# HuiGuanLab/Lite-MKD

Hardware: AMD Instinct MI355X
Metric: episodes/sec (5-way 5-shot, 8x224^2 frames) (higher is better)
Workload: dtype f32

## Files before the change

include/lmkd.h:

```cpp
#ifndef LMKD_H
#define LMKD_H
#ifdef __cplusplus
extern "C" {
#endif

int lmkd_abi_version(void);
const char* lmkd_last_error(void);
int lmkd_device_check(int device);
int lmkd_set_activation_dtype(int mode);
int lmkd_get_activation_dtype(void);

int lmkd_gemm_f32(char layA, char layB, int M, int N, int K, float alpha, const float* A, long lda, long sA,
                  const float* B, long ldb, long sB, float beta, float* C, long ldc, long sC, const float* bias,
                  int relu, int batch, void* stream);
int lmkd_gemm_set_mode(int mode);
int lmkd_gemm_set_tile(int t);
long lmkd_gemm_ticket_words(void);
int lmkd_gemm_f32_splitk(char layA, char layB, int M, int N, int K, float alpha, const float* A, long lda, long sA,
                         const float* B, long ldb, long sB, float beta, float* C, long ldc, long sC, const float* bias,
                         int relu, int batch, void* workspace, long ws_bytes, unsigned* tickets, void* stream);

long lmkd_conv2d_packed_weight_elems(int Cout, int Cin, int Cs, int KH, int KW, int mode);
int lmkd_conv2d_pack_weights(const float* w_oihw, float* wp, int Cout, int Cin, int Cs, int KH, int KW, int mode ,
                             void* stream);
int lmkd_conv2d_fwd_row_tiles(int N, int H, int W, int Cout, int KH, int KW, int stride, int pad);
int lmkd_conv2d_fwd_row_tiles_cs(int N, int H, int W, int Cs, int Cout, int KH, int KW, int stride, int pad);
int lmkd_set_elementwise_wg_per_cu(int n);
int lmkd_conv_set_compute_dtype(int mode);
typedef struct lmkd_amax_desc {
  const void* x_words;
  const void* dy_words;
  void* out_words;
  const void* ref_words;
  int flags;
} lmkd_amax_desc;
#define LMKD_AMAX_FENCED 1
int lmkd_h2_fence_eval(const void* const* words, void* const* refs, int n, int* flags, void* stream);
long lmkd_conv_h2_fallbacks(void);
int lmkd_amax(const float* x, long n, void* word, void* stream);
long lmkd_amax_words(void);
long lmkd_conv2d_plane_elems(int ncols, int Kp);
long lmkd_conv_h2_launches(void);
int lmkd_conv2d_repack_multi(const float* const* ws, void* const* wfs, const int* dims, int n, void* stream);
int lmkd_conv2d_split_weights(const float* wp, void* wf, int ncols, int Kp, void* stream);
int lmkd_conv_get_compute_dtype(void);
int lmkd_conv_set_wgrad_planes(int on);
int lmkd_conv_set_patch(int on);
int lmkd_conv_set_stem_patch(int on);
int lmkd_conv_set_s2_patch(int on);
int lmkd_conv_set_wgrad_win16(int on);
int lmkd_conv_set_wgrad_stem(int on);
int lmkd_conv_set_wgrad_window(int on);
int lmkd_conv_set_patch16(int on);
int lmkd_conv_set_persistent(int on);
int lmkd_conv_set_xcd_mode(int mode);
int lmkd_conv_set_tile(int id);
int lmkd_conv2d_fwd(const float* x, const float* wp_fwd, float* y, float* stat_partial, int N, int H, int W, int Cs, int Cout,
                    int KH, int KW, int stride, int pad, void* stream);
int lmkd_conv2d_fwd_pre(const float* x_raw, const float* pre_stats, const float* wp_fwd, float* y, float* stat_partial, int N, int H,
                        int W, int Cs, int Cout, int KH, int KW, int stride, int pad, void* stream);
int lmkd_conv2d_fwd_bn(const float* x, const float* wp_fwd, float* y, const float* bn_stats, const float* res , int relu,
                       int N, int H, int W, int Cs, int Cout, int KH, int KW, int stride, int pad, void* stream,
                       const lmkd_amax_desc* amax );
int lmkd_conv2d_bwd_data(const float* dy, const float* wp_dgrad, float* dx, int N, int H, int W, int Cin, int Cout, int KH, int KW,
                         int stride, int pad, int accumulate, void* stream);
int lmkd_conv2d_bwd_data_bn_tiles(int N, int H, int W, int Cin, int Cout, int KH, int KW, int stride, int pad);
int lmkd_conv2d_bwd_data_bn(const float* dy, const float* wp_dgrad, float* dx, const float* bn_x, const float* bn_stats, float* part,
                            int N, int H, int W, int Cin, int Cout, int KH, int KW, int stride, int pad, void* stream);
long lmkd_conv2d_bwd_weight_workspace(int N, int H, int W, int Cs, int Cout, int KH, int KW, int stride, int pad);
int lmkd_conv2d_bwd_weight(const float* x, const float* dy, float* dw_oihw, float* workspace, long ws_bytes, int N, int H, int W,
                           int Cs, int Cin, int Cout, int KH, int KW, int stride, int pad, void* stream);
int lmkd_conv2d_bwd_weight_pre(const float* x_raw, const float* pre_stats, const float* dy, float* dw_oihw, float* workspace,
                               long ws_bytes, int N, int H, int W, int Cs, int Cin, int Cout, int KH, int KW, int stride, int pad,
                               void* stream);

int lmkd_conv2d_plan(int kind, int N, int H, int W, int Cs, int Cin, int Cout, int KH, int KW, int stride, int pad, int* info_host);

int lmkd_conv2d_bwd_weight_acc(const float* x, const float* pre_stats, const float* dy, float* dw_oihw, float* workspace, long ws_bytes,
                               int N, int H, int W, int Cs, int Cin, int Cout, int KH, int KW, int stride, int pad, void* stream);

int lmkd_frames_u8_to_nhwc4(const unsigned char* src, float* dst, const int* crop_y, const int* crop_x, const int* flip, int F, int Hs,
                            int Ws, int H, int W, int frames_per_video, void* stream);
int lmkd_resize_plan(int in_size, int out_size, int* bounds_host, int* coeffs_host);
int lmkd_resize_pass_u8(const unsigned char* src, unsigned char* dst, const int* bounds_dev, const int* coeffs_dev, int ksize, long outer,
                        int n_in, int n_out, long inner, void* stream);
int lmkd_frames_resize_crop_nhwc4(const unsigned char* src, float* dst, const int* bounds_h, const int* coeffs_h, int ksize_h,
                                  const int* bounds_v, const int* coeffs_v, int ksize_v, const int* crop_y, const int* crop_x,
                                  const int* flip, int F, int Hs, int Ws, int Hr, int Wr, int H, int W, int frames_per_video, void* stream);
long lmkd_jpeg_desc_bytes(void);
long lmkd_jpeg_pool_bytes(int n);
const char* lmkd_jpeg_reason(int reason);
int lmkd_jpeg_plan(const unsigned char* data, const long long* offsets, int n, void* descs, void* pool, long pool_cap, long long* info,
                   long long* totals);
int lmkd_jpeg_decode(const unsigned char* data, const void* descs, const void* pool, int n, short* coef, unsigned char* planes,
                     unsigned char* out, int* status, long long max_blocks, long long max_pixels, void* stream);
int lmkd_jpeg_decode_host(const unsigned char* data, const void* descs, const void* pool, int n, short* coef, unsigned char* planes,
                          unsigned char* out, int* status);
int lmkd_nchw3_to_nhwc4(const float* x_nchw, float* y_nhwc4, int N, int H, int W, void* stream, void* amax_words);
long lmkd_ticket_words(void);
int lmkd_bn_finalize(const float* partial, int T, int C, long count, const float* gamma, const float* beta, float* running_mean,
                     float* running_var, float momentum, float eps, float* stats, double* scratch, unsigned* tickets, void* stream,
                     const lmkd_amax_desc* amax );
int lmkd_bn_running_update(float* running_mean, float* running_var, const float* stats, int C, float momentum, void* stream);
int lmkd_bn_running_update_multi(float* const* running_mean, float* const* running_var, const float* const* stats_first,
                                 const float* const* stats_second, const int* C, int n, float momentum, void* stream);
int lmkd_bn_running_update_multi_nbt(float* const* running_mean, float* const* running_var, const float* const* stats_first,
                                     const float* const* stats_second, long long* const* num_batches_tracked, const int* C, int n,
                                     float momentum, void* stream);
int lmkd_bn_eval_stats(int C, const float* gamma, const float* beta, const float* running_mean, const float* running_var, float eps,
                       float* stats, void* stream);
int lmkd_bn_apply(const float* x, const float* stats, const float* res, const float* rstats, float* y, long rows, int C, int relu,
                  int res_mode, unsigned* mask_bits, void* stream);
long lmkd_bn_bwd_workspace(int C);
int lmkd_bn_backward(const float* dy, const float* x, const float* yact, const float* stats, const float* gamma, float* dx,
                     float* g_out, float* dgamma, float* dbeta, float* coef, void* workspace, unsigned* tickets, long rows, int C,
                     int mask_mode, int accumulate_param_grads, void* stream);
int lmkd_bn_backward_part(const float* part, int T, const float* dy, const float* x, const float* stats, const float* gamma, float* dx,
                          float* dgamma, float* dbeta, float* coef, void* workspace, unsigned* tickets, long rows, int C,
                          int accumulate_param_grads, void* stream);
int lmkd_relu_backward(const float* dy, const float* y, float* g, long n, void* stream);
int lmkd_bn_relu_maxpool_fwd(const float* x, const float* stats, float* y, unsigned char* idx, float* cmax, int N, int H, int W, int C,
                             void* stream);
int lmkd_maxpool_bwd(const float* dy, const unsigned char* idx, float* g, int N, int H, int W, int C, void* stream);
int lmkd_bn_backward_stats(const float* dy, const float* cmax, const float* stats, const float* gamma, float* dgamma, float* dbeta,
                           float* coef, void* workspace, unsigned* tickets, long pooled_rows, long count, int C, int accumulate_param_grads,
                           void* stream);
int lmkd_stem_unpool_bn_bwd(const float* dy, const unsigned char* idx, const float* c, const float* stats, const float* coef, float* dc,
                            int N, int H, int W, int C, void* stream, const lmkd_amax_desc* amax );
int lmkd_adaptive_maxpool_mean_fwd(const float* x, float* y, int F, int H, int W, int C, void* stream);
int lmkd_adaptive_maxpool_mean_bwd(const float* x, const float* dy, float* dx, int F, int H, int W, int C, void* stream);
long lmkd_colsum_workspace(int C);
int lmkd_colsum(const float* a, const float* b, float* out, long rows, int C, int accumulate, void* workspace, unsigned* tickets,
                void* stream);

long lmkd_mnv3_stat_tiles(long pixels);
int lmkd_dw_conv_fwd(const float* x, const float* w, float* y, float* stat_partial, int N, int H, int W, int C, int K, int stride, void* stream);
int lmkd_dw_conv_bwd_data(const float* dy, const float* w, float* dx, int N, int H, int W, int C, int K, int stride, void* stream);
long lmkd_dw_conv_bwd_weight_workspace(int N, int H, int W, int C, int K, int stride);
int lmkd_dw_conv_bwd_weight(const float* x, const float* dy, float* dw, void* workspace, long ws_bytes, int N, int H, int W, int C, int K,
                            int stride, int accumulate, void* stream);
int lmkd_col_stats(const float* x, float* stat_partial, long rows, int C, void* stream);
int lmkd_bn_act_fwd(const float* x, const float* stats, const float* res, float* y, long rows, int C, int act, void* stream);
long lmkd_bn_act_bwd_workspace(long rows, int C);
int lmkd_bn_act_bwd(const float* dy, const float* x, const float* stats, const float* gamma, float* dx, float* dparams, void* workspace,
                    long ws_bytes, long rows, int C, int act, void* stream);
int lmkd_se_mean(const float* a, float* m, int N, int HW, int C, void* stream);
int lmkd_se_scale_fwd(const float* a, const float* s, float* y, int N, int HW, int C, void* stream);
int lmkd_se_scale_bwd(const float* dy, const float* a, const float* s, const float* dm, float* da, float* ds, int N, int HW, int C, void* stream);
int lmkd_hardsigmoid_fwd(const float* x, float* y, long n, void* stream);
int lmkd_hardsigmoid_bwd(const float* dy, const float* x, float* dx, long n, void* stream);
int lmkd_stem3x3_fwd(const float* x4, const float* w, float* y, float* stat_partial, int N, int H, int W, void* stream);
long lmkd_stem3x3_bwd_weight_workspace(int N, int H, int W);
int lmkd_stem3x3_bwd_weight(const float* x4, const float* dy, float* dw, void* workspace, long ws_bytes, int N, int H, int W, int accumulate,
                            void* stream);

int lmkd_dropout_mask(float* mask, long n, float p, unsigned long long seed, void* stream);
int lmkd_dropout_mask_dev(float* mask, long n, float p, const unsigned long long* seed_dev, void* stream);
int lmkd_add_pe(const float* x, const float* pe, const float* mask, float* y, long rows, int D, int L, void* stream);
int lmkd_mul(const float* a, const float* b, float* out, long n, void* stream);
int lmkd_axpby(const float* x, float* y, float alpha, float beta, long n, void* stream);
int lmkd_trx_tuple_ln_fwd(const float* P, const float* bk, const float* bv, const float* gamma, const float* beta, const int* rowmap,
                          float* Kn, float* Khat, float* V, float* rstd, int NV, int L, int D, float eps, void* stream);
int lmkd_layernorm_bwd_rows(float* dK_inout, const float* Khat, const float* rstd, const float* gamma, long rows, int D, void* stream);
int lmkd_trx_tuple_bwd_gather(const float* dKraw, const float* dV, const int* rowmap, float* dP, int NV, int L, int D, void* stream);
int lmkd_segment_softmax_fwd(float* S, long rows, long ld, int nseg, const int* seg_off, const int* seg_cnt, void* stream);
int lmkd_segment_softmax_bwd(const float* P, float* dP_inout, long rows, long ld, int nseg, const int* seg_off, const int* seg_cnt,
                             void* stream);
int lmkd_trx_dist_fwd(const float* Qv, const float* proto, float* logits, int Nq, int way, int T, int D, int nseg, const int* seg_col,
                      void* stream);
int lmkd_trx_dist_bwd(const float* Qv, float* proto_inout, const float* g, float* dQv, int Nq, int way, int T, int D, int nseg,
                      const int* seg_col, void* stream);
int lmkd_trx_sup_sim_fwd(const float* proto, const int* seg_col, float* sim, float* gram, int Nq, int way, int nseg, int T, int D,
                         void* stream);
int lmkd_trx_sup_sim_bwd(const float* proto, const int* seg_col, const float* gram, const float* dsim, float* dproto, int Nq, int way,
                         int nseg, int T, int D, void* stream);
long lmkd_supportdk_workspace(int way);
int lmkd_supportdk_fwd(const float* support, float* out, int way, int shot, int seq_len, int D, void* workspace, void* stream);
int lmkd_supportdk_bwd(const float* support, const float* g, float* dsupport, int way, int shot, int seq_len, int D, void* stream);
int lmkd_mean_frames(const float* x, float* y, long nv, int L, int D, void* stream);
int lmkd_mean_frames_bwd(const float* dy, float* dx, long nv, int L, int D, void* stream);
int lmkd_edist_fwd(const float* qm, const float* sm, const int* sup_class, float* dist, float* logits, int Nq, int Ns, int way, int D,
                   void* stream);
int lmkd_edist_bwd(const float* qm, const float* sm, const int* sup_class, const float* dist, const float* g, float* dqm, float* dsm,
                   int Nq, int Ns, int way, int D, void* stream);

int lmkd_layernorm_fwd(const float* x, const float* res, long res_rows, const float* gamma, const float* beta, float* y, long ldy,
                       long rows, int D, float eps, void* stream);
int lmkd_mha_small(const float* qkv, float* out, int B, int L, int D, int H, void* stream);

int lmkd_d2m_loss(const float* s_kl, const float* t_kl, const float* s_ce, const long long* labels, const float* s_sup,
                  const float* t_sup, int Rq, int C, int Rs, int Cs, float T, float w_kl, float w_sup, float w_ce, float* out4,
                  float* g_kl, float* g_ce, float* g_sup, void* stream);
long lmkd_mse_loss_workspace(void);
int lmkd_mse_loss(const float* s, const float* t, long n, float* out1, float* grad, void* workspace, void* stream);
int lmkd_accuracy(const float* l1, const float* l2, const long long* labels, long long* pred, float* acc, int R, int C, void* stream);
int lmkd_sgd_step(float* param, float* grad, float lr, long n, int zero_grad, void* stream);
int lmkd_adam_step(float* param, float* grad, float* exp_avg, float* exp_avg_sq, float lr, float beta1, float beta2, float eps,
                   long step, long n, int zero_grad, void* stream);
int lmkd_fill(float* p, float v, long n, void* stream);

int lmkd_conv2d_fwd_row_tiles_seg(int N, int H, int W, int Cs, int Cout, int KH, int KW, int stride, int pad, int seg_n0, int* tiles0 );
int lmkd_conv2d_fwd_seg(const float* x, const float* pre_stats , const float* wp, float* y,
                        float* stat_partial, int N, int H, int W, int Cs, int Cout, int KH, int KW, int stride, int pad, int seg_n0, void* stream,
                        const lmkd_amax_desc* amax );
int lmkd_conv2d_bwd_data_bn_tiles_seg(int N, int H, int W, int Cin, int Cout, int KH, int KW, int stride, int pad, int seg_n0, int* tiles0 );
// ... 47 lines not shown
```

lite-mkd_amd/csrc/capi.hip:

```cpp
#include "common.h"
#include <stdarg.h>

static thread_local char g_err[512] = "";

extern "C" void lmkd_set_error(const char* fmt, ...) {
  va_list ap;
  va_start(ap, fmt);
  vsnprintf(g_err, sizeof(g_err), fmt, ap);
  va_end(ap);
}

extern "C" const char* lmkd_last_error(void) { return g_err; }

extern "C" int lmkd_abi_version(void) { return 3; }

extern "C" int lmkd_device_check(int device) {
  hipDeviceProp_t p;
  hipError_t e = hipGetDeviceProperties(&p, device);
  if (e != hipSuccess) {
    lmkd_set_error("lmkd_device_check: %s", hipGetErrorString(e));
    return LMKD_EHIP;
  }
  if (strncmp(p.gcnArchName, "gfx950", 6) != 0) {
    lmkd_set_error("lmkd_device_check: device %d is %s, this library is built for gfx950 only", device, p.gcnArchName);
    return LMKD_EINVAL;
  }
  return LMKD_OK;
}

int g_lmkd_act_bf16 = 0;
extern "C" int lmkd_set_activation_dtype(int mode) {
  LMKD_REQUIRE(mode == 0 || mode == 1, "lmkd_set_activation_dtype: 0 = fp32, 1 = bf16");
  g_lmkd_act_bf16 = mode;
  return LMKD_OK;
}
extern "C" int lmkd_get_activation_dtype(void) { return g_lmkd_act_bf16; }
```

lite-mkd_amd/csrc/conv.hip:

```cpp
#include "gemm_core.h"
#include <atomic>
#include <mutex>

struct ConvGemmArgs {
  const float* src;
  const float* wpk;
  float* out;
  float* stat_partial;
  int N, Hs, Ws, Cs;
  int Hr, Wr, rows_per_class, tiles_per_class;
  int sh;
  int Ho, Wo, Co, omul;
  int Kp, cps, nclass;
  int n_rt, n_ct, xcd_mode;
  int taps_pm1;
  int grid_step;
  int grid_total;
  int same;
  int halo;
  int accum;
  const float* ep_stats;
  const float* ep_res;
  int ep_relu;
  const float* pre_stats;
// ... 1226 lines not shown
  ConvGemmArgs a;
  fwd_geometry(a, N, H, W, Cs, Cout, KH, KW, stride, pad, seg_n0);
  const ConvPlan p = plan_fwd(a, KH, KW, pad);
  if (tiles0) *tiles0 = p.seg_t0;
  return p.tiles_per_class;
}
extern "C" int lmkd_conv2d_fwd_row_tiles(int N, int H, int W, int Cout, int KH, int KW, int stride, int pad) {
  return lmkd_conv2d_fwd_row_tiles_cs(N, H, W, 32, Cout, KH, KW, stride, pad);
}

static int conv2d_fwd_impl(const float* x, const float* wp, float* y, float* stat_partial, const float* ep_stats,
                           const float* ep_res, int ep_relu, int N, int H, int W, int Cs, int Cout, int KH, int KW, int stride,
                           int pad, void* stream, const float* pre_stats = nullptr, int seg_n0 = 0, const lmkd_amax_desc* am = nullptr) {
  LMKD_REQUIRE(x && wp && y, "lmkd_conv2d_fwd: null pointer");
  if (seg_n0 <= 0 || seg_n0 >= N) seg_n0 = 0;
  LMKD_REQUIRE(!seg_n0 || (conv_planes() && !ep_stats), "lmkd_conv2d_fwd_seg: two frame segments exist in the bf16-plane modes (training / plain forward)");
  LMKD_REQUIRE(aligned16(x) && aligned16(wp), "lmkd_conv2d_fwd: x / packed weights must be 16-byte aligned");
  LMKD_REQUIRE(Cs % 32 == 0 || Cs == 4, "lmkd_conv2d_fwd: channel count %d must be 4 (padded stem) or a multiple of 32", Cs);
  LMKD_REQUIRE(N > 0 && H > 0 && W > 0 && Cout > 0, "lmkd_conv2d_fwd: empty tensor");
  const bool smallc = Cs == 4;
  const int KWp = kw_padded(Cs, KW);
  LMKD_REQUIRE(!smallc || KWp == 8, "lmkd_conv2d_fwd: padded-stem path needs KW <= 8");
  LMKD_REQUIRE(KH * (smallc ? 1 : KW) <= LMKD_MAX_TAPS, "lmkd_conv2d_fwd: kernel %dx%d has too many taps", KH, KW);
  LMKD_REQUIRE(H < 32768 && W < 32768, "lmkd_conv2d_fwd: spatial dims too large");
  const bool act16 = g_lmkd_act_bf16;
  LMKD_REQUIRE(!pre_stats || (stat_partial && !smallc && !act16),
               "lmkd_conv2d_fwd_pre: the fused BatchNorm+ReLU loader exists for the training forward with fp32 activations (stat_partial given, Cs %% 32 == 0)");
  LMKD_REQUIRE(!act16 || (conv_nprod() == 1 && !ep_stats), "bf16 activations need lmkd_conv_set_compute_dtype(1) (training / plain forward)");
  const int Ho = conv_out(H, KH, stride, pad), Wo = conv_out(W, KW, stride, pad);
  LMKD_REQUIRE(Ho > 0 && Wo > 0, "lmkd_conv2d_fwd: empty output");
  LMKD_REQUIRE((long)N * H * W * Cs < 2147483647L && (long)N * Ho * Wo * Cout < 2147483647L,
               "lmkd_conv2d_fwd: tensor exceeds 2^31 elements");
  LMKD_REQUIRE(!conv_planes() || (long)N * H * W * Cs * (act16 && Cs != 4 ? 2 : 4) < 0xffffffe0L,
               "lmkd_conv2d_fwd: input tensor exceeds the 4 GiB buffer range of the bf16-plane kernels");
  ConvGemmArgs a;
  fwd_geometry(a, N, H, W, Cs, Cout, KH, KW, stride, pad, seg_n0);
  a.src = x; a.wpk = wp; a.out = y; a.stat_partial = stat_partial;
  a.h2_xw = am ? (const unsigned*)am->x_words : nullptr;
  a.amax_out = am ? (unsigned*)am->out_words : nullptr;
  note_fenced(am);
  a.ep_stats = ep_stats; a.ep_res = ep_res; a.ep_relu = ep_relu;
  a.pre_stats = pre_stats;
  const ConvPlan p = plan_fwd(a, KH, KW, pad);
  if (p.src2) {
    LMKD_REQUIRE((long)N * H * W * Cs * 4 < 2147483647L, "lmkd_conv2d_fwd: input tensor exceeds the 2 GiB offset range of the stride-2 patch form");
    fwd_src2_args(a, W, KWp);
  }
  int rc = launch_conv(a, p, (hipStream_t)stream);
  if (rc == LMKD_OK && a.amax_out && p.amax_pass) {
    const long per = (long)Ho * Wo * Cout, n0 = seg_n0 ? seg_n0 * per : (long)N * per;
    rc = amax_impl(y, n0, a.amax_out, 1, stream, false);
    if (rc == LMKD_OK && seg_n0) rc = amax_impl(y + n0, (long)N * per - n0, a.amax_out + LMKD_AMAX_SEG_WORDS, 1, stream, false);
  }
  return rc;
}

extern "C" int lmkd_conv2d_fwd(const float* x, const float* wp, float* y, float* stat_partial, int N, int H, int W, int Cs,
                               int Cout, int KH, int KW, int stride, int pad, void* stream) {
  return conv2d_fwd_impl(x, wp, y, stat_partial, nullptr, nullptr, 0, N, H, W, Cs, Cout, KH, KW, stride, pad, stream);
}

extern "C" int lmkd_conv2d_fwd_seg(const float* x, const float* pre_stats, const float* wp, float* y, float* stat_partial, int N, int H, int W,
                                   int Cs, int Cout, int KH, int KW, int stride, int pad, int seg_n0, void* stream, const lmkd_amax_desc* amax) {
  return conv2d_fwd_impl(x, wp, y, stat_partial, nullptr, nullptr, 0, N, H, W, Cs, Cout, KH, KW, stride, pad, stream, pre_stats, seg_n0, amax);
}

extern "C" int lmkd_conv2d_fwd_pre(const float* x_raw, const float* pre_stats, const float* wp, float* y, float* stat_partial, int N,
                                   int H, int W, int Cs, int Cout, int KH, int KW, int stride, int pad, void* stream) {
  LMKD_REQUIRE(pre_stats, "lmkd_conv2d_fwd_pre: BatchNorm table of the input missing");
  return conv2d_fwd_impl(x_raw, wp, y, stat_partial, nullptr, nullptr, 0, N, H, W, Cs, Cout, KH, KW, stride, pad, stream, pre_stats);
}

extern "C" int lmkd_conv2d_fwd_bn(const float* x, const float* wp, float* y, const float* bn_stats, const float* res, int relu,
                                  int N, int H, int W, int Cs, int Cout, int KH, int KW, int stride, int pad, void* stream, const lmkd_amax_desc* amax) {
  LMKD_REQUIRE(bn_stats, "lmkd_conv2d_fwd_bn: BatchNorm table missing");
  LMKD_REQUIRE(!g_lmkd_act_bf16, "lmkd_conv2d_fwd_bn: fp32 tensors only (with bf16 tensors run lmkd_conv2d_fwd + lmkd_bn_apply)");
  LMKD_REQUIRE(!conv_planes() || Cs % 32 == 0, "lmkd_conv2d_fwd_bn: the bf16-plane modes need Cs %% 32 == 0 (Cs=%d)", Cs);
  return conv2d_fwd_impl(x, wp, y, nullptr, bn_stats, res, relu, N, H, W, Cs, Cout, KH, KW, stride, pad, stream, nullptr, 0, amax);
}

static int bwd_data_args(ConvGemmArgs& a, const float* dy, const float* wd, float* dx, int N, int H, int W, int Cin, int Cout, int KH, int KW,
                         int stride, int pad, int accumulate, int seg_n0 = 0, const lmkd_amax_desc* am = nullptr) {
  if (seg_n0 <= 0 || seg_n0 >= N) seg_n0 = 0;
  LMKD_REQUIRE(!seg_n0 || conv_planes(), "lmkd_conv2d_bwd_data_seg: two frame segments exist in the bf16-plane modes");
  LMKD_REQUIRE(Cout % 32 == 0, "lmkd_conv2d_bwd_data: Cout=%d must be a multiple of 32", Cout);
  LMKD_REQUIRE(stride == 1 || stride == 2, "lmkd_conv2d_bwd_data: stride %d unsupported", stride);
  LMKD_REQUIRE(KH * KW <= LMKD_MAX_TAPS, "lmkd_conv2d_bwd_data: kernel too large");
  LMKD_REQUIRE(!g_lmkd_act_bf16 || conv_nprod() == 1, "bf16 activations need lmkd_conv_set_compute_dtype(1)");
  const int Ho = conv_out(H, KH, stride, pad), Wo = conv_out(W, KW, stride, pad);
  LMKD_REQUIRE((long)N * H * W * Cin < 2147483647L && (long)N * Ho * Wo * Cout < 2147483647L,
               "lmkd_conv2d_bwd_data: tensor exceeds 2^31 elements");
  LMKD_REQUIRE(!conv_planes() || (long)N * Ho * Wo * Cout * (g_lmkd_act_bf16 ? 2 : 4) < 0xffffffe0L,
               "lmkd_conv2d_bwd_data: dy exceeds the 4 GiB buffer range of the bf16-plane kernels");
  dgrad_geometry(a, N, H, W, Cin, Cout, KH, KW, stride, pad, seg_n0);
  a.src = dy; a.wpk = wd; a.out = dx; a.accum = accumulate;
  a.h2_xw = am ? (const unsigned*)am->dy_words : nullptr;
  return LMKD_OK;
}

extern "C" int lmkd_conv2d_bwd_data(const float* dy, const float* wd, float* dx, int N, int H, int W, int Cin, int Cout,
                                    int KH, int KW, int stride, int pad, int accumulate, void* stream) {
  LMKD_REQUIRE(dy && wd && dx, "lmkd_conv2d_bwd_data: null pointer");
  LMKD_REQUIRE(aligned16(dy) && aligned16(wd), "lmkd_conv2d_bwd_data: operands must be 16-byte aligned");
  ConvGemmArgs a;
  if (const int rc = bwd_data_args(a, dy, wd, dx, N, H, W, Cin, Cout, KH, KW, stride, pad, accumulate)) return rc;
  return launch_conv(a, plan_dgrad(a), (hipStream_t)stream);
}

extern "C" int lmkd_conv2d_bwd_data_bn_tiles_seg(int N, int H, int W, int Cin, int Cout, int KH, int KW, int stride, int pad, int seg_n0, int* tiles0) {
  if (stride != 1 || Cout % 32 != 0 || KH * KW > LMKD_MAX_TAPS) return 0;
  ConvGemmArgs a;
  if (bwd_data_args(a, nullptr, nullptr, nullptr, N, H, W, Cin, Cout, KH, KW, stride, pad, 0, seg_n0)) return 0;
  const ConvPlan p = plan_dgrad(a);
  if (!p.bnb_form) return 0;
  if (tiles0) *tiles0 = p.seg_t0;
  return p.tiles_per_class;
}
extern "C" int lmkd_conv2d_bwd_data_bn_tiles(int N, int H, int W, int Cin, int Cout, int KH, int KW, int stride, int pad) {
  return lmkd_conv2d_bwd_data_bn_tiles_seg(N, H, W, Cin, Cout, KH, KW, stride, pad, 0, nullptr);
}
extern "C" int lmkd_conv2d_bwd_data_seg(const float* dy, const float* wd, float* dx, const float* bn_x, const float* bn_stats, float* part, int N,
                                        int H, int W, int Cin, int Cout, int KH, int KW, int stride, int pad, int accumulate, int seg_n0, void* stream,
                                        const lmkd_amax_desc* amax) {
  LMKD_REQUIRE(dy && wd && dx, "lmkd_conv2d_bwd_data_seg: null pointer");
  LMKD_REQUIRE(aligned16(dy) && aligned16(wd), "lmkd_conv2d_bwd_data_seg: operands must be 16-byte aligned");
  LMKD_REQUIRE((bn_x != nullptr) == (bn_stats != nullptr) && (bn_x != nullptr) == (part != nullptr), "lmkd_conv2d_bwd_data_seg: bn_x, bn_stats and part go together");
  ConvGemmArgs a;
  if (const int rc = bwd_data_args(a, dy, wd, dx, N, H, W, Cin, Cout, KH, KW, stride, pad, accumulate, seg_n0, amax)) return rc;
  note_fenced(amax);
  if (bn_x) {
    LMKD_REQUIRE(!accumulate && aligned16(bn_x) && aligned16(bn_stats), "lmkd_conv2d_bwd_data_seg: the fused BatchNorm sums need a plain (non-accumulating) launch and aligned operands");
    a.bnb_x = bn_x; a.bnb_stats = bn_stats; a.stat_partial = part;
  }
  const ConvPlan p = plan_dgrad(a);
  LMKD_REQUIRE(!bn_x || p.bnb_form, "lmkd_conv2d_bwd_data_seg: this launch has no fused form (lmkd_conv2d_bwd_data_bn_tiles_seg returned 0)");
  return launch_conv(a, p, (hipStream_t)stream);
}
extern "C" int lmkd_conv2d_bwd_data_bn(const float* dy, const float* wd, float* dx, const float* bn_x, const float* bn_stats, float* part,
                                       int N, int H, int W, int Cin, int Cout, int KH, int KW, int stride, int pad, void* stream) {
  LMKD_REQUIRE(dy && wd && dx && bn_x && bn_stats && part, "lmkd_conv2d_bwd_data_bn: null pointer");
  LMKD_REQUIRE(aligned16(dy) && aligned16(wd) && aligned16(bn_x) && aligned16(bn_stats), "lmkd_conv2d_bwd_data_bn: operands must be 16-byte aligned");
  ConvGemmArgs a;
  if (const int rc = bwd_data_args(a, dy, wd, dx, N, H, W, Cin, Cout, KH, KW, stride, pad, 0)) return rc;
  a.bnb_x = bn_x; a.bnb_stats = bn_stats; a.stat_partial = part;
  const ConvPlan p = plan_dgrad(a);
  LMKD_REQUIRE(p.bnb_form, "lmkd_conv2d_bwd_data_bn: this launch has no fused form (lmkd_conv2d_bwd_data_bn_tiles returned 0)");
  return launch_conv(a, p, (hipStream_t)stream);
}

static int g_wgrad_planes = 1;
extern "C" int lmkd_conv_set_wgrad_planes(int on) { g_wgrad_planes = on ? 1 : 0; return LMKD_OK; }
static int g_wgrad_win16 = 1;
extern "C" int lmkd_conv_set_wgrad_win16(int on) { g_wgrad_win16 = on ? 1 : 0; return LMKD_OK; }
static int g_wgrad_window = 1;
extern "C" int lmkd_conv_set_wgrad_window(int on) { g_wgrad_window = on < 0 ? 0 : on; return LMKD_OK; }
static inline bool wgrad_win_eligible(int W, int Cs, int Cout, int KH, int KW, int stride, int pad) {
  return g_wgrad_window && g_wgrad_planes && conv_planes() && KH == 3 && KW == 3 && stride == 1 && pad == 1 &&
         Cs % 32 == 0 && 32 + 2 * (W + 1) <= 256;
}
static void wgrad_win_plan(int Mpix, int W, int Cs, int Cout, int* cob, int* splits, int* steps_per_split) {
  *cob = Cout >= 128 ? 4 : 2;
  const int tiles = cdiv(Cout, 32 * *cob) * (Cs / 32);
  const int steps = cdiv(Mpix, LMKD_BK);
  const int warm = cdiv(2 * (W + 1), LMKD_BK);
  const int resident = 256 * ((conv_nprod() >= 6 && *cob == 2) ? 2 : 8 / *cob);
  int sp = g_wgrad_window > 1 ? cdiv(g_wgrad_window, tiles)
                              : std::max((int)(((long)resident * steps + 19600L * 4 / *cob) / (39200L * 4 / *cob)), cdiv(128, tiles));
  const int cap = std::max(1, steps / (12 * warm));
  if (sp > cap) sp = cap;
  *steps_per_split = cdiv(steps, sp);
  *splits = cdiv(steps, *steps_per_split);
}

static void wgrad_plan(int Mpix, int Cout, int Kp, int* splits, int* steps_per_split, int* bm, int* bn, bool planes = false) {
  *bm = Cout <= 64 ? 64 : 128;
  *bn = (Kp % 128 == 0 && Kp >= 1024) ? 128 : 64;
  int per_cu = (*bm == 128 && *bn == 128) ? 2 : ((*bm == 64 && *bn == 64) ? 4 : 3);
  if (planes) {
    if (*bm == 64 && *bn == 128) *bn = 64;
    const int npl = conv_nprod() == 1 ? 1 : 3;
    const long lds = 1L * npl * LMKD_BK * ((*bm * 2 + 64) + (*bn * 2 + 64));
    per_cu = (int)(160 * 1024 / lds);
    if (per_cu > 4) per_cu = 4;
    if (per_cu < 1) per_cu = 1;
  }
  const int tiles = cdiv(Cout, *bm) * cdiv(Kp, *bn);
  const int steps = cdiv(Mpix, LMKD_BK);
  const int slots = 256 * per_cu;
  int best_sp = 1;
  double best_cost = 1e30;
  for (int r = 1; r <= 3; ++r) {
    int sp = (slots * r) / tiles;
    if (sp > steps / 4) sp = steps / 4;
    if (sp < 1) sp = 1;
    const int sps = cdiv(steps, sp);
    sp = cdiv(steps, sps);
    const double rounds = (double)cdiv((long)tiles * sp, slots);
    const double cost = rounds * sps + 1.0 * sp / 8.0;
    if (cost < best_cost) { best_cost = cost; best_sp = sp; }
  }
  if (planes && *bm == 64 && *bn == 64 && best_sp < cdiv(steps, 64)) best_sp = cdiv(steps, 64);
  *steps_per_split = cdiv(steps, best_sp);
  *splits = cdiv(steps, *steps_per_split);
}

static int g_wgrad_stem = 1;
extern "C" int lmkd_conv_set_wgrad_stem(int on) { g_wgrad_stem = on ? 1 : 0; return LMKD_OK; }
static int stem_wgrad_plan(int N, int H, int W, int Cs, int Cout, int KH, int KW, int stride, int pad, int* G) {
  if (!g_wgrad_stem || !g_wgrad_planes || conv_nprod(g_lmkd_act_bf16) < 6 || Cs != 4 || Cout != 64 || KH != 7 || KW != 7 || stride != 2 || pad != 3) return 0;
  const int Ho = conv_out(H, KH, stride, pad), Wo = conv_out(W, KW, stride, pad);
  if (Wo < 17 || Wo > 128 || W > 2 * Wo || Ho < 1) return 0;
  const int units = N * cdiv(Ho, 2);
  int g = std::max(1, 2048 / (2 * Wo));
  g = std::min(g, std::max(1, units / 256));
  *G = g;
  return cdiv(units, g);
}

enum class WgFam : unsigned char {
  Stem,
  Win16,
  Win,
  Planes,
  Tile,
};
struct WgradPlan {
  WgFam fam;
  bool pre, act16, smallc;
  int nprod;
  int bm, bn;
  int cob;
  int G;
  int splits, splits0, sps0, sps1, seg_pix0;
  int xcd;
  int grid;
  long need;
  long ws;
};

static long wgrad_workspace(int N, int H, int W, int Cs, int Cout, int KH, int KW, int stride, int pad) {
  const int Ho = conv_out(H, KH, stride, pad), Wo = conv_out(W, KW, stride, pad);
  const int Kp = KH * kw_padded(Cs, KW) * Cs;
  int G, splits, sps, bm, bn;
  if (const int slabs = stem_wgrad_plan(N, H, W, Cs, Cout, KH, KW, stride, pad, &G)) return (long)slabs * Cout * Kp * sizeof(float);
  wgrad_plan(N * Ho * Wo, Cout, Kp, &splits, &sps, &bm, &bn, conv_planes() && g_wgrad_planes);
  if (wgrad_win_eligible(W, Cs, Cout, KH, KW, stride, pad)) {
    int cob, wsplits, wsps;
    wgrad_win_plan(N * Ho * Wo, W, Cs, Cout, &cob, &wsplits, &wsps);
    splits = std::max(splits, wsplits);
  }
  return (long)splits * Cout * Kp * sizeof(float);
}

static WgradPlan plan_wgrad(int N, int H, int W, int Cs, int Cout, int KH, int KW, int stride, int pad, int seg_n0, bool pre, bool maxima) {
  WgradPlan p;
  memset(&p, 0, sizeof(p));
  const bool act16 = g_lmkd_act_bf16;
  const int Ho = conv_out(H, KH, stride, pad), Wo = conv_out(W, KW, stride, pad);
  const int Kp = KH * kw_padded(Cs, KW) * Cs, Mpix = N * Ho * Wo;
  p.pre = pre; p.act16 = act16; p.smallc = Cs == 4;
  p.ws = wgrad_workspace(N, H, W, Cs, Cout, KH, KW, stride, pad);
  if (seg_n0)
    p.ws = std::max(p.ws, wgrad_workspace(seg_n0, H, W, Cs, Cout, KH, KW, stride, pad) + wgrad_workspace(N - seg_n0, H, W, Cs, Cout, KH, KW, stride, pad));
  p.seg_pix0 = seg_n0 ? seg_n0 * Ho * Wo : Mpix;
  if (const int slabs = stem_wgrad_plan(N, H, W, Cs, Cout, KH, KW, stride, pad, &p.G)) {
    p.fam = WgFam::Stem;
    p.nprod = conv_nprod(false, maxima);
    p.splits = p.grid = slabs;
  } else if (wgrad_win_eligible(W, Cs, Cout, KH, KW, stride, pad)) {
    const bool w16 = g_wgrad_win16 && conv_nprod(act16) >= 6;
    p.fam = w16 ? WgFam::Win16 : WgFam::Win;
    p.nprod = w16 ? conv_nprod(false, maxima) : conv_nprod(act16);
    wgrad_win_plan(Mpix, W, Cs, Cout, &p.cob, &p.splits, &p.sps0);
    p.splits0 = p.splits;
    if (seg_n0) {
      int sp1, cob1;
      wgrad_win_plan(p.seg_pix0, W, Cs, Cout, &p.cob, &p.splits0, &p.sps0);
      wgrad_win_plan(Mpix - p.seg_pix0, W, Cs, Cout, &cob1, &sp1, &p.sps1);
      p.splits = p.splits0 + sp1;
    }
    p.grid = 8 * cdiv(p.splits, 8) * cdiv(Cout, 32 * p.cob) * (Cs / 32);
  } else {
    const bool planes = conv_planes() && g_wgrad_planes;
    p.fam = planes ? WgFam::Planes : WgFam::Tile;
    p.nprod = planes ? conv_nprod(act16, maxima && !p.smallc && !pre) : (conv_nprod() == 1 ? 1 : 0);
    wgrad_plan(Mpix, Cout, Kp, &p.splits, &p.sps0, &p.bm, &p.bn, planes);
    p.splits0 = p.splits;
    if (seg_n0) {
      int sp1, bm1, bn1;
      wgrad_plan(p.seg_pix0, Cout, Kp, &p.splits0, &p.sps0, &p.bm, &p.bn, planes);
      wgrad_plan(Mpix - p.seg_pix0, Cout, Kp, &sp1, &p.sps1, &bm1, &bn1, planes);
      p.splits = p.splits0 + sp1;
    }
    p.xcd = (g_xcd_mode != 0 && g_xcd_mode != 1 && p.splits >= 32) ? 1 : 0;
    p.grid = (p.xcd ? 8 * cdiv(p.splits, 8) : p.splits) * cdiv(Cout, p.bm) * cdiv(Kp, p.bn);
  }
  p.need = (long)p.splits * Cout * Kp * sizeof(float);
  return p;
}

template <int NPROD, int D, int RLC>
static void launch_stem_wgrad(const StemWgradArgs& w, dim3 grid, size_t lds, hipStream_t s) {
  lds_attr_once<stem_wgrad_kernel<NPROD, D, RLC>>(160 * 1024);
  hipLaunchKernelGGL((stem_wgrad_kernel<NPROD, D, RLC>), grid, dim3(512), lds, s, w);
}
template <int NPROD>
static void launch_stem_wgrad(const StemWgradArgs& w, dim3 grid, size_t lds, hipStream_t s) {
  const bool deep = cdiv(2 * w.Wo, 32) >= 6;
  if (deep && w.RL == 1856) launch_stem_wgrad<NPROD, 6, 1856>(w, grid, lds, s);
  else if (deep) launch_stem_wgrad<NPROD, 6, 0>(w, grid, lds, s);
  else launch_stem_wgrad<NPROD, 2, 0>(w, grid, lds, s);
}
template <int COB>
static void launch_wgrad_win(const WgradWinArgs& w, const WgradPlan& p, bool big, hipStream_t s) {
  const dim3 grid(p.grid);
  if (p.fam == WgFam::Win16) {
    constexpr int JW = COB == 2 ? 1 : 2;
    constexpr int NT = 64 * COB * (2 / JW);
    with_nprod<3, 6, 9>(p.nprod, [&](auto np) {
      if (big && p.pre) hipLaunchKernelGGL((conv_wgrad_win16_kernel<COB, np, 256, true, 9, JW>), grid, dim3(NT), 0, s, w);
      else if (big) hipLaunchKernelGGL((conv_wgrad_win16_kernel<COB, np, 256, false, 9, JW>), grid, dim3(NT), 0, s, w);
      else if (p.pre) hipLaunchKernelGGL((conv_wgrad_win16_kernel<COB, np, 128, true, 9, JW>), grid, dim3(NT), 0, s, w);
      else hipLaunchKernelGGL((conv_wgrad_win16_kernel<COB, np, 128, false, 9, JW>), grid, dim3(NT), 0, s, w);
    });
    return;
  }
  auto go = [&](auto np, auto a16, auto pre) {
    constexpr int NPROD = decltype(np)::value;
    constexpr bool A16 = decltype(a16)::value, PRE = decltype(pre)::value;
    constexpr int TPW = (COB == 2 && NPROD != 1) ? 5 : 9;
    constexpr int NT = 64 * COB * ((9 + TPW - 1) / TPW);
    if (big) hipLaunchKernelGGL((conv_wgrad_win_kernel<COB, NPROD, A16, 256, PRE, TPW>), grid, dim3(NT), 0, s, w);
    else hipLaunchKernelGGL((conv_wgrad_win_kernel<COB, NPROD, A16, 128, PRE, TPW>), grid, dim3(NT), 0, s, w);
  };
  using T = std::true_type;
  using F = std::false_type;
  if (p.act16) go(std::integral_constant<int, 1>{}, T{}, F{});
  else with_nprod<1, 6, 9>(p.nprod, [&](auto np) { if (p.pre) go(np, F{}, T{}); else go(np, F{}, F{}); });
}

template <class CFG>
static void launch_wgrad_planes(const WgradArgs& a, const WgradPlan& p, hipStream_t s) {
  const dim3 grid(p.grid), block(256);
  if (p.act16) {
    if (p.smallc) hipLaunchKernelGGL((conv_wgrad_x3_kernel<CFG, true, 1, false, true>), grid, block, 0, s, a);
    else hipLaunchKernelGGL((conv_wgrad_x3_kernel<CFG, false, 1, false, true>), grid, block, 0, s, a);
  } else if (p.smallc) {
    with_nprod<1, 6, 9>(p.nprod, [&](auto np) { hipLaunchKernelGGL((conv_wgrad_x3_kernel<CFG, true, np, false>), grid, block, 0, s, a); });
  } else if (p.pre) {
    with_nprod<1, 6, 9>(p.nprod, [&](auto np) { hipLaunchKernelGGL((conv_wgrad_x3_kernel<CFG, false, np, true>), grid, block, 0, s, a); });
  } else {
    with_nprod<1, 3, 6, 9>(p.nprod, [&](auto np) { hipLaunchKernelGGL((conv_wgrad_x3_kernel<CFG, false, np, false>), grid, block, 0, s, a); });
  }
}

template <class CFG, bool SM, int THR>
static void launch_wgrad_tile(const WgradArgs& a, const WgradPlan& p, hipStream_t s) {
  const dim3 grid(p.grid);
  if (p.nprod == 1) hipLaunchKernelGGL((conv_wgrad_kernel<CFG, SM, true>), grid, dim3(THR), 0, s, a);
  else if (!SM && p.pre) hipLaunchKernelGGL((conv_wgrad_kernel<CFG, false, false, true>), grid, dim3(THR), 0, s, a);
  else hipLaunchKernelGGL((conv_wgrad_kernel<CFG, SM, false>), grid, dim3(THR), 0, s, a);
}

static int conv2d_bwd_weight_impl(const float* x, const float* pre_stats, const float* dy, float* dw_oihw, float* workspace,
                                  long ws_bytes, int N, int H, int W, int Cs, int Cin, int Cout, int KH, int KW, int stride, int pad,
                                  void* stream, int accumulate = 0, int seg_n0 = 0, const lmkd_amax_desc* am = nullptr) {
  const unsigned* amax_x = am ? (const unsigned*)am->x_words : nullptr;
  const unsigned* amax_dy = am ? (const unsigned*)am->dy_words : nullptr;
  note_fenced(am);
  LMKD_REQUIRE(x && dy && dw_oihw && workspace, "lmkd_conv2d_bwd_weight: null pointer");
  if (seg_n0 <= 0 || seg_n0 >= N) seg_n0 = 0;
  LMKD_REQUIRE(aligned16(x) && aligned16(dy) && aligned16(workspace), "lmkd_conv2d_bwd_weight: operands must be 16-byte aligned");
  LMKD_REQUIRE(Cs % 32 == 0 || Cs == 4, "lmkd_conv2d_bwd_weight: channel count %d must be 4 or a multiple of 32", Cs);
  LMKD_REQUIRE(Cout % 4 == 0, "lmkd_conv2d_bwd_weight: Cout %% 4 != 0");
  const bool smallc = Cs == 4;
  const WgradPlan p = plan_wgrad(N, H, W, Cs, Cout, KH, KW, stride, pad, seg_n0, pre_stats != nullptr, amax_x && amax_dy);
  LMKD_REQUIRE(!seg_n0 || p.fam != WgFam::Tile, "lmkd_conv2d_bwd_weight_seg: two frame segments exist in the bf16-plane modes");
  LMKD_REQUIRE(!pre_stats || (!smallc && (conv_nprod() != 1 || p.fam != WgFam::Tile) && !p.act16), "lmkd_conv2d_bwd_weight_pre: Cs %% 32 == 0, fp32 activations only");
  LMKD_REQUIRE(!p.act16 || (conv_nprod() == 1 && p.fam != WgFam::Tile), "bf16 activations need lmkd_conv_set_compute_dtype(1) and the plane weight-gradient kernel");
  const int Ho = conv_out(H, KH, stride, pad), Wo = conv_out(W, KW, stride, pad);
  const int KWp = kw_padded(Cs, KW), Kp = KH * KWp * Cs, Mpix = N * Ho * Wo;
  LMKD_REQUIRE((long)N * H * W * Cs < 2147483647L && (long)Mpix * Cout < 2147483647L, "lmkd_conv2d_bwd_weight: tensor too large");
  LMKD_REQUIRE(ws_bytes >= p.need, "lmkd_conv2d_bwd_weight: workspace too small");
  hipStream_t s = (hipStream_t)stream;
  if (p.fam == WgFam::Stem) {
    LMKD_REQUIRE((long)Mpix * 64 * 4 < 0xffffffe0L && (long)N * H * W * 16 < 0xffffffe0L, "lmkd_conv2d_bwd_weight: tensor too large for 32-bit byte offsets");
    StemWgradArgs w;
    memset(&w, 0, sizeof(w));
    w.dy = dy; w.x = x; w.slab = workspace;
    w.h2_xw = amax_x; w.h2_dyw = amax_dy;
    w.N = N; w.H = H; w.W = W; w.Ho = Ho; w.Wo = Wo;
    w.upi = cdiv(Ho, 2); w.units = N * w.upi; w.G = p.G; w.slabs = p.splits;
    w.RL = 16 * Wo + 64;
    const size_t lds = (size_t)2 * 10 * 3 * w.RL + 2 * 3 * STEM_WG_APLANE;
    with_nprod<3, 6, 9>(p.nprod, [&](auto np) { launch_stem_wgrad<np>(w, dim3(p.grid), lds, s); });
    LMKD_CHECK_LAUNCH("stem_wgrad_kernel");
    if (Kp <= 256) {
      hipLaunchKernelGGL(wgrad_reduce_stem_kernel, dim3(Cout), dim3(256, 4), 0, s, (const float*)workspace, dw_oihw, p.splits, Cout, Cin, Cs, KH, KW,
                         KWp, Kp, accumulate);
    } else {
      launch_wgrad_reduce((const float*)workspace, dw_oihw, p.splits, Cout, Cin, Cs, KH, KW, KWp, Kp, accumulate, s);
    }
    LMKD_CHECK_LAUNCH("wgrad_reduce_kernel");
    return LMKD_OK;
  }
  if (p.fam == WgFam::Win16 || p.fam == WgFam::Win) {
    LMKD_REQUIRE((long)Mpix * std::max(Cs, Cout) * 4 < 2147483647L, "lmkd_conv2d_bwd_weight: tensor too large for 32-bit byte offsets");
    WgradWinArgs w;
    memset(&w, 0, sizeof(w));
    w.dy = dy; w.x = x; w.slab = workspace; w.pre_stats = pre_stats;
    w.h2_xw = amax_x; w.h2_dyw = amax_dy;
    w.N = N; w.H = H; w.W = W; w.Cs = Cs; w.Co = Cout; w.Kp = Kp; w.Mpix = Mpix;
    w.steps_total = cdiv(Mpix, LMKD_BK);
    w.splits = p.splits; w.steps_per_split = p.sps0;
    w.seg_pix0 = p.seg_pix0; w.seg_splits0 = p.splits0; w.sps1 = p.sps1;
    w.n_ct = cdiv(Cout, 32 * p.cob); w.n_it = Cs / 32;
    w.div_hw = make_fastdiv(H * W); w.div_w = make_fastdiv(W);
    const bool big = 32 + 2 * (W + 1) > 128;
    if (p.cob == 4) launch_wgrad_win<4>(w, p, big, s);
    else launch_wgrad_win<2>(w, p, big, s);
    LMKD_CHECK_LAUNCH("conv_wgrad_win_kernel");
    launch_wgrad_reduce((const float*)workspace, dw_oihw, p.splits, Cout, Cin, Cs, KH, KW, KWp, Kp, accumulate, s);
    LMKD_CHECK_LAUNCH("wgrad_reduce_kernel");
    return LMKD_OK;
  }
  WgradArgs a;
  memset(&a, 0, sizeof(a));
  a.dy = dy; a.x = x; a.slab = workspace; a.pre_stats = pre_stats;
  a.h2_xw = amax_x; a.h2_dyw = amax_dy;
  a.N = N; a.Hs = H; a.Ws = W; a.Cs = Cs;
  a.Ho = Ho; a.Wo = Wo; a.Co = Cout;
  a.stride = stride; a.pad = pad; a.KH = KH; a.KW = KW; a.KWp = KWp;
  a.Kp = Kp; a.Mpix = Mpix;
  a.steps_per_split = p.sps0;
  a.seg_pix0 = p.seg_pix0; a.seg_splits0 = p.splits0; a.sps1 = p.sps1;
  a.steps_total = cdiv(Mpix, LMKD_BK);
  a.div_hw = make_fastdiv(Ho * Wo); a.div_w = make_fastdiv(Wo);
  a.n_mt = cdiv(Cout, p.bm); a.n_jt = cdiv(Kp, p.bn); a.splits = p.splits;
  a.xcd_mode = p.xcd;
  const int bm = p.bm, bn = p.bn;
  LMKD_REQUIRE(!smallc || (bm == 64 && bn == 64), "lmkd_conv2d_bwd_weight: padded-stem path expects Cout <= 64");
  if (p.fam == WgFam::Planes) {
    if (bm == 128 && bn == 128) launch_wgrad_planes<WgCfg<128, 128, 2, 2>>(a, p, s);
    else if (bm == 128) launch_wgrad_planes<WgCfg<128, 64, 2, 2>>(a, p, s);
    else launch_wgrad_planes<WgCfg<64, 64, 2, 2>>(a, p, s);
    LMKD_CHECK_LAUNCH("conv_wgrad_x3_kernel");
  } else {
    if (smallc) launch_wgrad_tile<TileCfg<64, 64, 2, 2>, true, LMKD_THREADS>(a, p, s);
    else if (bm == 64 && bn == 64) launch_wgrad_tile<TileCfg<64, 64, 2, 2>, false, LMKD_THREADS>(a, p, s);
    else if (bm == 128 && bn == 64) launch_wgrad_tile<TileCfg<128, 64, 2, 2>, false, LMKD_THREADS>(a, p, s);
    else if (bm == 64 && bn == 128) launch_wgrad_tile<TileCfg<64, 128, 2, 2>, false, LMKD_THREADS>(a, p, s);
    else launch_wgrad_tile<TileCfg<128, 128, 2, 4>, false, 512>(a, p, s);
    LMKD_CHECK_LAUNCH("conv_wgrad_kernel");
  }
  launch_wgrad_reduce((const float*)workspace, dw_oihw, p.splits, Cout, Cin, Cs, KH, KW, KWp, Kp, accumulate, s);
  LMKD_CHECK_LAUNCH("wgrad_reduce_kernel");
  return LMKD_OK;
}

extern "C" long lmkd_conv2d_bwd_weight_workspace_seg(int N, int H, int W, int Cs, int Cout, int KH, int KW, int stride, int pad, int seg_n0) {
  if (seg_n0 <= 0 || seg_n0 >= N) seg_n0 = 0;
  return plan_wgrad(N, H, W, Cs, Cout, KH, KW, stride, pad, seg_n0, false, false).ws;
}
extern "C" long lmkd_conv2d_bwd_weight_workspace(int N, int H, int W, int Cs, int Cout, int KH, int KW, int stride, int pad) {
  return lmkd_conv2d_bwd_weight_workspace_seg(N, H, W, Cs, Cout, KH, KW, stride, pad, 0);
}

extern "C" int lmkd_conv2d_bwd_weight(const float* x, const float* dy, float* dw_oihw, float* workspace, long ws_bytes,
                                      int N, int H, int W, int Cs, int Cin, int Cout, int KH, int KW, int stride, int pad,
                                      void* stream) {
  return conv2d_bwd_weight_impl(x, nullptr, dy, dw_oihw, workspace, ws_bytes, N, H, W, Cs, Cin, Cout, KH, KW, stride, pad, stream);
}

extern "C" int lmkd_conv2d_bwd_weight_pre(const float* x_raw, const float* pre_stats, const float* dy, float* dw_oihw,
                                          float* workspace, long ws_bytes, int N, int H, int W, int Cs, int Cin, int Cout, int KH,
                                          int KW, int stride, int pad, void* stream) {
  LMKD_REQUIRE(pre_stats, "lmkd_conv2d_bwd_weight_pre: BatchNorm table of the input missing");
  return conv2d_bwd_weight_impl(x_raw, pre_stats, dy, dw_oihw, workspace, ws_bytes, N, H, W, Cs, Cin, Cout, KH, KW, stride, pad, stream);
}

extern "C" int lmkd_conv2d_bwd_weight_acc(const float* x, const float* pre_stats, const float* dy, float* dw_oihw, float* workspace,
                                          long ws_bytes, int N, int H, int W, int Cs, int Cin, int Cout, int KH, int KW, int stride,
                                          int pad, void* stream) {
  return conv2d_bwd_weight_impl(x, pre_stats, dy, dw_oihw, workspace, ws_bytes, N, H, W, Cs, Cin, Cout, KH, KW, stride, pad, stream, 1);
}


extern "C" int lmkd_conv2d_bwd_weight_seg(const float* x, const float* pre_stats, const float* dy, float* dw_oihw, float* workspace, long ws_bytes,
                                          int N, int H, int W, int Cs, int Cin, int Cout, int KH, int KW, int stride, int pad, int accumulate,
                                          int seg_n0, void* stream, const lmkd_amax_desc* amax) {
  return conv2d_bwd_weight_impl(x, pre_stats, dy, dw_oihw, workspace, ws_bytes, N, H, W, Cs, Cin, Cout, KH, KW, stride, pad, stream, accumulate, seg_n0, amax);
}

extern "C" int lmkd_conv2d_plan(int kind, int N, int H, int W, int Cs, int Cin, int Cout, int KH, int KW, int stride, int pad,
                                int* info) {
  LMKD_REQUIRE(info && kind >= 0 && kind <= 2, "lmkd_conv2d_plan: kind must be 0 (forward), 1 (data gradient) or 2 (weight gradient)");
  LMKD_REQUIRE(N > 0 && H > 0 && W > 0 && Cout > 0 && KH > 0 && KW > 0 && stride > 0, "lmkd_conv2d_plan: bad shape");
  if (kind == 2) {
    const WgradPlan p = plan_wgrad(N, H, W, Cs, Cout, KH, KW, stride, pad, 0, false, false);
    info[1] = p.xcd; info[2] = p.splits; info[3] = p.grid;
    switch (p.fam) {
      case WgFam::Stem: info[0] = 14; info[4] = 2; break;
      case WgFam::Win16:
      case WgFam::Win: info[0] = p.cob == 4 ? 5 : 6; info[1] = 1; info[4] = 1; break;
      default: info[0] = (p.bm == 128 && p.bn == 128) ? 1 : (p.bm == 128 ? 2 : (p.bn == 128 ? 4 : 3)); info[4] = 0; break;
    }
    return LMKD_OK;
  }
  ConvGemmArgs a;
  if (kind == 0) fwd_geometry(a, N, H, W, Cs, Cout, KH, KW, stride, pad, 0);
  else dgrad_geometry(a, N, H, W, Cin, Cout, KH, KW, stride, pad, 0);
  const ConvPlan p = kind == 0 ? plan_fwd(a, KH, KW, pad) : plan_dgrad(a);
  info[0] = p.tile; info[1] = p.xcd; info[2] = p.nclass; info[3] = p.grid;
  info[4] = p.fam == ConvFam::Stem ? 2 : (p.fam == ConvFam::Patch || p.fam == ConvFam::Patch16 || p.fam == ConvFam::Patch1p ? 1 : 0);
  return LMKD_OK;
}
```

lite-mkd_amd/csrc/conv_patch.h:

```cpp
#pragma once

#define PATCH_HALO_MAX 57

template <int NPL> struct PatchRow { static constexpr int BYTES = NPL == 1 ? 80 : (NPL == 2 ? 144 : 208); };

static inline size_t patch_lds_bytes(int bm, int halo, int npl) { return (size_t)(bm + 2 * halo + 1) * (npl == 1 ? 80 : (npl == 2 ? 144 : 208)); }

#ifdef LMKD_STAMPS
__device__ unsigned long long g_lmkd_stamps[4096 * 8];
#define STAMP(k) do { if (threadIdx.x == 0 && (blockIdx.x & 63) == 0 && (blockIdx.x >> 6) < 4096) g_lmkd_stamps[(blockIdx.x >> 6) * 8 + (k)] = __builtin_amdgcn_s_memtime(); } while (0)
#else
#define STAMP(k) do { } while (0)
#endif


template <class Cfg>
__device__ __forceinline__ void patch_h2_epilogue(const ConvGemmArgs& a, f32x16 (&acc)[Cfg::TM][Cfg::TN], const int* s_out, float* s_red, int rt,
                                                  int n0, int wm, int wn, int lane, int tid, int seg, int row0, int M, float h2_ix, float h2_iw) {
  const int cl0 = wn * (Cfg::TN * 32) + (lane & 31);
  const bool bnb = a.bnb_x != nullptr;
  float s1[Cfg::TN], s2[Cfg::TN];
  float amo = 0.f;
  const bool plain = a.nclass == 1;
  const int rows = M - row0 < Cfg::BM ? M - row0 : Cfg::BM;
// ... 170 lines not shown
  if (Lc < 0) return;
  u32x4 rp[NI];
  float4 psc = float4(), psh = float4();
  auto issue_patch = [&](const PatchTile& d, int cc) {
#pragma unroll
    for (int i = 0; i < NI; ++i)
      if (i * RPP < P) rp[i] = __builtin_amdgcn_raw_buffer_load_b128(prs, ((d.p_ok >> i) & 1u) ? d.p_off0 + i * p_step + (unsigned)(cc * 32 * ESZ) : X3_OOB, 0, 0);
    if (PRE) {
      const float* pre_tab = a.pre_stats + (long)d.seg * 5 * a.Cs;
      psc = *reinterpret_cast<const float4*>(pre_tab + 2 * a.Cs + cc * 32 + pk);
      psh = *reinterpret_cast<const float4*>(pre_tab + 3 * a.Cs + cc * 32 + pk);
    }
  };
  for (int j = tid; j < ROWB / 4; j += Cfg::THREADS) reinterpret_cast<unsigned*>(psm + (long)P * ROWB)[j] = 0u;
  int it = 0;
  bool requested = false;
  for (;;) {
    PSTAMP(0);
    const int Ln = PERSIST ? next_tile(Lc + a.grid_step, nxt) : -1;
    const int ntap = cur.ntap;
    const Tap* taps = s_args.taps[cur.cls];
    const int ph = cur.cls >> 1, pw = cur.cls & 1;
    const int M = cur.mend, row0 = cur.row0, n0 = cur.ct * Cfg::BN;
    const int nk = ntap * a.cps;
    const Tap my_tap = taps[lane < ntap ? lane : 0];
    if (!requested && nk > 0) issue_patch(cur, 0);
    requested = false;
    unsigned h2_xbits = 0u, h2_wbits = 0u;
    if constexpr (NPROD == 3) {
      h2_xbits = a.h2_xw[cur.seg * LMKD_AMAX_SEG_WORDS + (tid & (LMKD_AMAX_SLOTS - 1)) * LMKD_AMAX_STRIDE];
      h2_wbits = *reinterpret_cast<const unsigned*>(reinterpret_cast<const unsigned short*>(a.wpk) + (long)a.Co * a.Kp * 16);
    }
    LB lb;
    const bool neg = NPL == 3 && NPROD != 3 && x3_neg_tile(cur.ltile, cur.ltiles);
    if constexpr (NPROD == 3)
      lb.init(reinterpret_cast<const unsigned short*>(a.wpk) + (long)a.Co * a.Kp * 16 + 32, a.Co, a.Kp, n0 + wn * (Cfg::TN * 32), lane, false);
    else
      lb.init(a.wpk, a.Co, a.Kp, n0 + wn * (Cfg::TN * 32), lane, neg);
    u32x4 rb0[LB::NR], rb1[LB::NR];
    int b_tp = 0, b_cc = 0;
    if (nk > 0) {
      lb.load(__builtin_amdgcn_readlane(my_tap.kofs, 0), rb0);
      if (++b_tp == ntap) { b_tp = 0; ++b_cc; }
      if (nk > 1) {
        lb.load((ntap > 1 ? __builtin_amdgcn_readlane(my_tap.kofs, 1) : __builtin_amdgcn_readlane(my_tap.kofs, 0)) + b_cc * LMKD_BK, rb1);
        if (++b_tp == ntap) { b_tp = 0; ++b_cc; }
      }
    }
    const bool inv = PERSIST && a.nclass == 1;
    const bool tables = !inv || it == 0;
    if (tables && tid < ntap) {
      s_tap_shift[tid] = (my_tap.dh * a.Ws + my_tap.dw) * ROWB;
      s_tap_kofs[tid] = my_tap.kofs;
      s_tap_dhw[tid] = (my_tap.dh << 16) | (my_tap.dw & 0xffff);
    }
    if (tables && NPROD == 3 && a.taps_pm1 && tid < 64) {
      const int rb = tid & 7, cb = tid >> 3;
      unsigned m = 0;
      for (int tp = 0; tp < ntap; ++tp) {
        const int dh = taps[tp].dh, dw = taps[tp].dw;
        if (((rb >> (dh + 1)) & 1) && ((cb >> (dw + 1)) & 1)) m |= 1u << tp;
      }
      s_mask_lut[tid] = (unsigned short)m;
    }
    if (a.nclass != 1 || !(NPROD == 3)) {
      for (int r = tid; r < Cfg::BM; r += Cfg::THREADS) {
        const int m = row0 + r;
        int ob = -1;
        if (m < M) {
          if (a.nclass == 1) {
            ob = m * a.Co;
          } else {
            const int n = fdiv(m, a.div_hw);
            const int rem = m - n * a.Hs * a.Ws;
            const int aa = fdiv(rem, a.div_w), bb = rem - aa * a.Ws;
            const int oh = aa * a.omul + ph, ow = bb * a.omul + pw;
            if (oh < a.Ho && ow < a.Wo) ob = ((n * a.Ho + oh) * a.Wo + ow) * a.Co;
          }
        }
        s_out[r] = ob;
      }
    }
    if (tables) __syncthreads();
    unsigned a_base[Cfg::TM], a_mask[Cfg::TM];
    {
      int hh[Cfg::TM], ww[Cfg::TM];
#pragma unroll
      for (int i = 0; i < Cfg::TM; ++i) {
        const int r = a_row + 32 * i, m = row0 + r;
        a_base[i] = (unsigned)((r + halo) * ROWB + 16 * h);
        a_mask[i] = 0;
        hh[i] = -0x4000; ww[i] = 0;
        if (m < M) {
          const int n = fdiv(m, a.div_hw);
          const int rem = m - n * a.Hs * a.Ws;
          hh[i] = fdiv(rem, a.div_w);
          ww[i] = rem - hh[i] * a.Ws;
        }
      }
      if (NPROD == 3 && a.taps_pm1) {
#pragma unroll
        for (int i = 0; i < Cfg::TM; ++i) {
          const unsigned Hs = (unsigned)a.Hs, Ws = (unsigned)a.Ws;
          const unsigned rbits = ((unsigned)(hh[i] - 1) < Hs ? 1u : 0u) | ((unsigned)hh[i] < Hs ? 2u : 0u) | ((unsigned)(hh[i] + 1) < Hs ? 4u : 0u);
          const unsigned cbits = ((unsigned)(ww[i] - 1) < Ws ? 1u : 0u) | ((unsigned)ww[i] < Ws ? 2u : 0u) | ((unsigned)(ww[i] + 1) < Ws ? 4u : 0u);
          a_mask[i] = s_mask_lut[rbits | (cbits << 3)];
        }
      } else
      for (int t0 = 0; t0 < ntap; t0 += 9) {
        int dv[9];
#pragma unroll
        for (int q = 0; q < 9; ++q) dv[q] = s_tap_dhw[t0 + q < ntap ? t0 + q : 0];
#pragma unroll
        for (int q = 0; q < 9; ++q) {
          const int dh = dv[q] >> 16, dw = (int)(short)(dv[q] & 0xffff);
#pragma unroll
          for (int i = 0; i < Cfg::TM; ++i) {
            const int y = hh[i] + dh, x = ww[i] + dw;
            if (t0 + q < ntap && (unsigned)y < (unsigned)a.Hs && (unsigned)x < (unsigned)a.Ws) a_mask[i] |= 1u << (t0 + q);
          }
        }
      }
    }
    float h2_sx = 1.f, h2_ix = 1.f, h2_iw = 1.f;
    if constexpr (NPROD == 3) {
      unsigned v = h2_xbits;
#pragma unroll
      for (int o = 32; o >= 1; o >>= 1) {
        const unsigned u = (unsigned)__shfl_xor((int)v, o, 64);
        v = u > v ? u : v;
      }
      h2_sx = h2_scale(__builtin_amdgcn_readfirstlane(v));
      h2_ix = 1.f / h2_sx;
      h2_iw = 1.f / h2_scale(h2_wbits);
    }
    auto store_patch = [&]() {
#pragma unroll
      for (int i = 0; i < NI; ++i) {
        const int j = tid / LPR + RPP * i;
        if (j >= P) continue;
        unsigned char* d = psm + j * ROWB + pk * 2;
        if constexpr (IN16) {
          *reinterpret_cast<u32x4*>(d) = rp[i];
        } else {
          float4 v = make_float4(__uint_as_float(rp[i].x), __uint_as_float(rp[i].y), __uint_as_float(rp[i].z), __uint_as_float(rp[i].w));
          if (PRE && ((cur.p_ok >> i) & 1u)) {
            v.x = fmaxf(fmaf(v.x, psc.x, psh.x), 0.f); v.y = fmaxf(fmaf(v.y, psc.y, psh.y), 0.f);
            v.z = fmaxf(fmaf(v.z, psc.z, psh.z), 0.f); v.w = fmaxf(fmaf(v.w, psc.w, psh.w), 0.f);
          }
          if (NPL == 1) {
            *reinterpret_cast<uint2*>(d) = x3_round4(v);
          } else if constexpr (NPROD == 3) {
            uint2 q0, q1;
            h2_split4(v, h2_sx, q0, q1);
            *reinterpret_cast<uint2*>(d) = q0;
            *reinterpret_cast<uint2*>(d + 64) = q1;
          } else {
            uint2 q0, q1, q2;
            x3_split4(v, q0, q1, q2);
            *reinterpret_cast<uint2*>(d) = q0;
            *reinterpret_cast<uint2*>(d + 64) = q1;
            *reinterpret_cast<uint2*>(d + 128) = q2;
          }
        }
      }
    };
    f32x16 acc[Cfg::TM][Cfg::TN];
#pragma unroll
    for (int i = 0; i < Cfg::TM; ++i)
#pragma unroll
      for (int j = 0; j < Cfg::TN; ++j)
#pragma unroll
        for (int e = 0; e < 16; ++e) acc[i][j][e] = 0.f;
    auto issue_b = [&](u32x4 (&rb)[LB::NR]) {
      lb.load(s_tap_kofs[b_tp] + b_cc * LMKD_BK, rb);
      if (++b_tp == ntap) { b_tp = 0; ++b_cc; }
    };
    int k_tp = 0, k_cc = 0;
    constexpr bool PIPE = NPL == 1;
    bf16x8 avp0[2][NPL][Cfg::TM], avp1[2][NPL][Cfg::TM];
    auto read_tap = [&](int tp, bf16x8 (&dst)[2][NPL][Cfg::TM]) {
      const unsigned sh = (unsigned)s_tap_shift[tp];
#pragma unroll
      for (int i = 0; i < Cfg::TM; ++i) {
        const unsigned ad = ((a_mask[i] >> tp) & 1u) ? a_base[i] + sh : zero_addr;
#pragma unroll
        for (int g = 0; g < 2; ++g)
#pragma unroll
          for (int p = 0; p < NPL; ++p) dst[g][p][i] = *reinterpret_cast<const bf16x8*>(psm + ad + p * 64 + g * 32);
      }
    };
    auto step = [&](int t, u32x4 (&rb)[LB::NR], u32x4 (&rbn)[LB::NR], bf16x8 (&avc)[2][NPL][Cfg::TM], bf16x8 (&avn)[2][NPL][Cfg::TM]) {
      if (k_tp == 0) {
        if (!(inv && k_cc == 0)) __syncthreads();
        store_patch();
        __syncthreads();
        {
          const bool more = k_cc + 1 < a.cps;
          const bool ahead = PERSIST && !more && Ln >= 0 && nxt.ntap > 0;
          if (more || ahead) {
            PatchTile d;
            d.p_off0 = more ? cur.p_off0 : nxt.p_off0;
            d.p_ok = more ? cur.p_ok : nxt.p_ok;
            d.seg = more ? cur.seg : nxt.seg;
            issue_patch(d, more ? k_cc + 1 : 0);
            requested = ahead;
          }
        }
        if constexpr (PIPE) read_tap(0, avc);
      }
      if constexpr (PIPE) {
        if (k_tp + 1 < ntap) read_tap(k_tp + 1, avn);
        __builtin_amdgcn_sched_barrier(0);
#pragma unroll
        for (int g = 0; g < 2; ++g)
#pragma unroll
          for (int j = 0; j < Cfg::TN; ++j) {
            const bf16x8 b0 = x3_as_bf16(rb[j * 2 + g]);
#pragma unroll
            for (int i = 0; i < Cfg::TM; ++i) acc[i][j] = __builtin_amdgcn_mfma_f32_32x32x16_bf16(avc[g][0][i], b0, acc[i][j], 0, 0, 0);
          }
        if (++k_tp == ntap) { k_tp = 0; ++k_cc; }
        __builtin_amdgcn_sched_barrier(0);
        x3_landed(rbn);
        x3_landed(rp);
        __builtin_amdgcn_sched_barrier(0);
        if (t + 2 < nk) issue_b(rb);
        return;
      }
      const unsigned sh = (unsigned)s_tap_shift[k_tp];
      unsigned ad[Cfg::TM];
#pragma unroll
      for (int i = 0; i < Cfg::TM; ++i) ad[i] = ((a_mask[i] >> k_tp) & 1u) ? a_base[i] + sh : zero_addr;
      constexpr bool AHEAD = NPL * Cfg::TM < 12 && (Cfg::THREADS == 512 || NPL == 1);
      bf16x8 av[2][NPL][Cfg::TM];
      auto read_a = [&](int g) {
#pragma unroll
        for (int p = 0; p < NPU; ++p)
#pragma unroll
          for (int i = 0; i < Cfg::TM; ++i) av[AHEAD ? g : 0][p][i] = *reinterpret_cast<const bf16x8*>(psm + ad[i] + p * 64 + g * 32);
      };
      read_a(0);
      if (AHEAD) read_a(1);
      __builtin_amdgcn_sched_barrier(0);
#pragma unroll
      for (int g = 0; g < 2; ++g) {
        const int ga = AHEAD ? g : 0;
        if (!AHEAD && g == 1) {
          __builtin_amdgcn_sched_barrier(0);
          read_a(1);
          __builtin_amdgcn_sched_barrier(0);
        }
#pragma unroll
        for (int j = 0; j < Cfg::TN; ++j) {
          if constexpr (NPROD == 1) {
            const bf16x8 b0 = x3_as_bf16(rb[j * 2 + g]);
#pragma unroll
            for (int i = 0; i < Cfg::TM; ++i) acc[i][j] = __builtin_amdgcn_mfma_f32_32x32x16_bf16(av[ga][0][i], b0, acc[i][j], 0, 0, 0);
          } else if constexpr (NPROD == 3) {
            const f16x8 b0 = __builtin_bit_cast(f16x8, rb[j * 4 + g * 2 + 0]), b1 = __builtin_bit_cast(f16x8, rb[j * 4 + g * 2 + 1]);
#pragma unroll
            for (int i = 0; i < Cfg::TM; ++i) {
              f32x16 c = acc[i][j];
              c = __builtin_amdgcn_mfma_f32_32x32x16_f16(__builtin_bit_cast(f16x8, av[ga][0][i]), b1, c, 0, 0, 0);
              c = __builtin_amdgcn_mfma_f32_32x32x16_f16(__builtin_bit_cast(f16x8, av[ga][1][i]), b0, c, 0, 0, 0);
              c = __builtin_amdgcn_mfma_f32_32x32x16_f16(__builtin_bit_cast(f16x8, av[ga][0][i]), b0, c, 0, 0, 0);
              acc[i][j] = c;
            }
          } else {
            const bf16x8 b0 = x3_as_bf16(rb[j * 6 + g * 3 + 0]), b1 = x3_as_bf16(rb[j * 6 + g * 3 + 1]), b2 = x3_as_bf16(rb[j * 6 + g * 3 + 2]);
#pragma unroll
            for (int i = 0; i < Cfg::TM; ++i) {
              f32x16 c = acc[i][j];
              if (NPROD == 9) {
                c = __builtin_amdgcn_mfma_f32_32x32x16_bf16(av[ga][2][i], b2, c, 0, 0, 0);
                c = __builtin_amdgcn_mfma_f32_32x32x16_bf16(av[ga][1][i], b2, c, 0, 0, 0);
                c = __builtin_amdgcn_mfma_f32_32x32x16_bf16(av[ga][2][i], b1, c, 0, 0, 0);
              }
              c = __builtin_amdgcn_mfma_f32_32x32x16_bf16(av[ga][1][i], b1, c, 0, 0, 0);
              c = __builtin_amdgcn_mfma_f32_32x32x16_bf16(av[ga][0][i], b2, c, 0, 0, 0);
              c = __builtin_amdgcn_mfma_f32_32x32x16_bf16(av[ga][2][i], b0, c, 0, 0, 0);
              c = __builtin_amdgcn_mfma_f32_32x32x16_bf16(av[ga][0][i], b1, c, 0, 0, 0);
              c = __builtin_amdgcn_mfma_f32_32x32x16_bf16(av[ga][1][i], b0, c, 0, 0, 0);
              c = __builtin_amdgcn_mfma_f32_32x32x16_bf16(av[ga][0][i], b0, c, 0, 0, 0);
              acc[i][j] = c;
            }
          }
        }
      }
      if (++k_tp == ntap) { k_tp = 0; ++k_cc; }
      __builtin_amdgcn_sched_barrier(0);
      x3_landed(rbn);
      x3_landed(rp);
      __builtin_amdgcn_sched_barrier(0);
      if (t + 2 < nk) issue_b(rb);
    };
    PSTAMP(1);
    if (nk > 0) {
      x3_landed(rp);
      x3_landed(rb0);
      x3_landed(rb1);
      __builtin_amdgcn_sched_barrier(0);
      PSTAMP(2);
      int t = 0;
      for (; t + 1 < nk; t += 2) {
        step(t, rb0, rb1, avp0, avp1);
        step(t + 1, rb1, rb0, avp1, avp0);
// ... 18 lines not shown
```

lite-mkd_amd/csrc/conv_patch16.h:

```cpp
#pragma once
#ifndef LMKD_ABL
#define LMKD_ABL 0
#endif

__device__ __host__ __forceinline__ constexpr int patch16_kslot(int q) { return ((q & 1) << 1) | (q >> 1); }
__device__ __forceinline__ int patch16_pixel(int j) { return (j >= 4 && j < 12) ? 2 * (j - 4) : (j < 4 ? 2 * j + 1 : 2 * (j - 8) + 1); }

template <int CTRL>
__device__ __forceinline__ float dpp_add(float v) {
  return v + __int_as_float(__builtin_amdgcn_update_dpp(0, __float_as_int(v), CTRL, 0xf, 0xf, false));
}
__device__ __forceinline__ float row16_sum(float v) {
  v = dpp_add<0xB1>(v);
  v = dpp_add<0x4E>(v);
  v = dpp_add<0x141>(v);
  return dpp_add<0x140>(v);
}

template <int TN, int NPW = 3>
struct X3FragB16 {
  static constexpr int NT = 2 * TN;
  static constexpr int NR = NT * NPW;
  __amdgpu_buffer_rsrc_t rs;
  unsigned off[NT];
// ... 114 lines not shown
  constexpr int NPL = 3;
  constexpr int NPU = NPROD == 3 ? 2 : 3;
  constexpr int ROWB = PatchRow<NPL>::BYTES;
  constexpr int LPR = 8;
  constexpr int RPP = Cfg::THREADS / LPR;
  constexpr int NI = (Cfg::BM + 2 * PATCH_HALO_MAX + RPP - 1) / RPP;
  constexpr int NB = 2 * Cfg::TM, NC = 2 * Cfg::TN;
  using LB = X3FragB16<Cfg::TN, NPU>;
  extern __shared__ __attribute__((aligned(16))) unsigned char psm[];
  __shared__ int s_out[Cfg::BM];
  __shared__ int s_tap_kofs[LMKD_MAX_TAPS];
  static_assert(NB == 4 && PatchRow<NPL>::BYTES % 16 == 0 && PatchRow<NPL>::BYTES / 16 * (Cfg::BM + 2 * PATCH_HALO_MAX + 1) < 65536,
                "four 16-bit patch offsets (in units of 16 bytes) per lane and tap");
  __shared__ __attribute__((aligned(8))) unsigned short s_adp[LMKD_MAX_TAPS * Cfg::BM];
  __shared__ float s_red[Cfg::WM * Cfg::BN * 2];
  __shared__ int s_src[SRC2 ? Cfg::BM + 2 * PATCH_HALO_MAX : 1];
  const int tid = threadIdx.x;
  STAMP(0);
  int rt, ct;
  if (!xcd_decode(blockIdx.x, a.n_rt, a.n_ct, a.xcd_mode, rt, ct)) return;
  const int tile = rt / a.nclass;
  const int cls = rt - tile * a.nclass;
  const int ph = cls >> 1, pw = cls & 1;
  const int ntap = a.ntap[cls];
  if (a.accum && ntap == 0) return;
  const Tap* taps = a.taps[cls];
  const int halo = a.halo, P = Cfg::BM + 2 * halo;
  const SegTile sg = seg_tile(a, tile, Cfg::BM);
  const int M = sg.mend;
  const int row0 = sg.row0, n0 = ct * Cfg::BN;
  if (tid < ntap) {
    const Tap tp = taps[tid];
    s_tap_kofs[tid] = tp.kofs;
  }
  for (int r = tid; r < Cfg::BM; r += Cfg::THREADS) {
    const int m = row0 + r;
    int ob = -1;
    if (m < M) {
      if (a.nclass == 1) {
        ob = m * a.Co;
      } else {
        const int n = fdiv(m, a.div_hw);
        const int rem = m - n * a.Hs * a.Ws;
        const int aa = fdiv(rem, a.div_w), bb = rem - aa * a.Ws;
        const int oh = aa * a.omul + ph, ow = bb * a.omul + pw;
        if (oh < a.Ho && ow < a.Wo) ob = ((n * a.Ho + oh) * a.Wo + ow) * a.Co;
      }
    }
    s_out[r] = ob;
  }
  for (int j = tid; j < ROWB / 4; j += Cfg::THREADS) reinterpret_cast<unsigned*>(psm + (long)P * ROWB)[j] = 0u;
  if constexpr (SRC2) {
    for (int j = tid; j < P; j += Cfg::THREADS) {
      const int m = row0 - halo + j;
      int off = -1;
      if (m >= 0 && m < a.rows_per_class) {
        const int n = fdiv(m, a.div_hw);
        const int rem = m - n * a.Hs * a.Ws;
        const int aa = fdiv(rem, a.div_w), bb = rem - aa * a.Ws;
        off = (((n * 2 * a.Hs + 2 * aa) * a.s2_wfull + 2 * bb) * a.Cs) * 4;
      }
      s_src[j] = off;
    }
  }
  const int lane = tid & 63, wave = tid >> 6;
  float h2_sx = 1.f, h2_ix = 1.f, h2_iw = 1.f;
  bool h2_one = true;
  if constexpr (NPROD == 3) {
    h2_sx = h2_scale(amax_read(a.h2_xw, sg.seg));
    const float sw = h2_scale(*reinterpret_cast<const unsigned*>(reinterpret_cast<const unsigned short*>(a.wpk) + (long)a.Co * a.Kp * 16));
    h2_ix = 1.f / h2_sx;
    h2_iw = 1.f / sw;
    const int ex = (int)((__float_as_uint(h2_ix) >> 23) & 0xffu) + (int)((__float_as_uint(h2_iw) >> 23) & 0xffu) - 254;
    h2_one = ex >= -126 && ex <= 126;
    if (h2_one) h2_ix *= h2_iw;
  }
  const int wm = wave / Cfg::WN, wn = wave % Cfg::WN;
  const int kq = lane >> 4;
  const int ksl = patch16_kslot(kq);
  const int pxl = patch16_pixel(lane & 15);
  constexpr bool EARLY = !SRC2 && Cfg::BN == 64;
  if constexpr (!EARLY) {
    for (int r = tid; r < Cfg::BM; r += Cfg::THREADS) {
      const int m = row0 + r;
      const int within = r % (Cfg::TM * 32), px = within & 15;
      const int l16 = (px & 1) ? ((px >> 1) + (px < 8 ? 0 : 8)) : (px >> 1) + 4;
      unsigned short* dst = s_adp + ((r / (Cfg::TM * 32)) * 16 + l16) * NB + (within >> 4);
      int hh = -0x40000000, ww = 0;
      if (m < M) {
        const int n = fdiv(m, a.div_hw);
        const int rem = m - n * a.Hs * a.Ws;
        hh = fdiv(rem, a.div_w);
        ww = rem - hh * a.Ws;
      }
      for (int tp = 0; tp < ntap; ++tp) {
        const int y = hh + taps[tp].dh, x = ww + taps[tp].dw;
        const bool in = (unsigned)y < (unsigned)a.Hs && (unsigned)x < (unsigned)a.Ws;
        dst[tp * Cfg::BM] = (unsigned short)((in ? (r + halo + taps[tp].dh * a.Ws + taps[tp].dw) : P) * (ROWB / 16));
      }
    }
  }
  const unsigned lane_off = (unsigned)(16 * ksl);
  const unsigned short* adp_lane = s_adp + (wm * 16 + (lane & 15)) * NB;
  const __amdgpu_buffer_rsrc_t prs = x3_rsrc(a.src, (long)a.N * a.Hs * a.Ws * a.Cs * 4 * (SRC2 ? 4 : 1));
  const int pk = (tid & (LPR - 1)) * 4;
  const long pix0 = (long)row0 - halo + tid / LPR;
  const unsigned p_off0 = (unsigned)((pix0 * a.Cs + pk) * 4), p_step = (unsigned)(RPP * a.Cs * 4);
  unsigned p_ok = 0;
#pragma unroll
  for (int i = 0; i < NI; ++i) {
    const long pix = pix0 + RPP * i;
    if (tid / LPR + RPP * i < P && pix >= 0 && pix < (long)a.N * a.Hs * a.Ws) p_ok |= 1u << i;
  }
  u32x4 rp[NI];
  int k_cc_abl = 0;
  float4 psc = float4(), psh = float4();
  const float* pre_tab = PRE ? a.pre_stats + (long)sg.seg * 5 * a.Cs : nullptr;
  auto issue_patch = [&](int cc, int sc = 0) {
    if ((LMKD_ABL & 32) && cc > 0) return;
    if constexpr (SRC2) {
      const unsigned rel = (unsigned)((a.s2_off[sc] + cc * 32 + pk) * 4);
#pragma unroll
      for (int i = 0; i < NI; ++i) {
        if (i * RPP >= P) continue;
        const int j = tid / LPR + RPP * i;
        const int so = j < P ? s_src[j] : -1;
        rp[i] = __builtin_amdgcn_raw_buffer_load_b128(prs, so >= 0 ? (unsigned)so + rel : X3_OOB, 0, 0);
      }
      return;
    }
#pragma unroll
    for (int i = 0; i < NI; ++i)
      if (i * RPP < P) rp[i] = __builtin_amdgcn_raw_buffer_load_b128(prs, ((p_ok >> i) & 1u) ? p_off0 + i * p_step + (unsigned)(cc * 32 * 4) : X3_OOB, 0, 0);
    if (PRE) {
      psc = *reinterpret_cast<const float4*>(pre_tab + 2 * a.Cs + cc * 32 + pk);
      psh = *reinterpret_cast<const float4*>(pre_tab + 3 * a.Cs + cc * 32 + pk);
    }
  };
  auto store_patch = [&]() {
    if ((LMKD_ABL & 64) && k_cc_abl > 0) return;
#pragma unroll
    for (int i = 0; i < NI; ++i) {
      const int j = tid / LPR + RPP * i;
      if (j >= P) continue;
      unsigned char* d = psm + j * ROWB + pk * 2;
      float4 v = make_float4(__uint_as_float(rp[i].x), __uint_as_float(rp[i].y), __uint_as_float(rp[i].z), __uint_as_float(rp[i].w));
      if (PRE && ((p_ok >> i) & 1u)) {
        v.x = fmaxf(fmaf(v.x, psc.x, psh.x), 0.f); v.y = fmaxf(fmaf(v.y, psc.y, psh.y), 0.f);
        v.z = fmaxf(fmaf(v.z, psc.z, psh.z), 0.f); v.w = fmaxf(fmaf(v.w, psc.w, psh.w), 0.f);
      }
      uint2 q0, q1, q2;
      if constexpr (NPROD == 3) {
        if (LMKD_ABL & 4) { q0 = make_uint2(__float_as_uint(v.x), __float_as_uint(v.y)); q1 = make_uint2(__float_as_uint(v.z), __float_as_uint(v.w)); }
        else h2_split4(v, h2_sx, q0, q1);
      } else x3_split4(v, q0, q1, q2);
      *reinterpret_cast<uint2*>(d) = q0;
      *reinterpret_cast<uint2*>(d + 64) = q1;
      if (NPU == 3) *reinterpret_cast<uint2*>(d + 128) = q2;
    }
  };
  const bool neg = x3_neg_tile(sg.ltile, sg.ltiles);
  if (NPROD == 3 && neg) h2_ix = -h2_ix;
  LB lb;
  lb.init(a.wpk, a.Co, a.Kp, n0 + wn * (Cfg::TN * 32), lane, neg);
  f32x4 acc[NB][NC];
#pragma unroll
  for (int b = 0; b < NB; ++b)
#pragma unroll
    for (int c = 0; c < NC; ++c) acc[b][c] = f32x4{0.f, 0.f, 0.f, 0.f};
  const int nk = ntap * a.cps;
  u32x4 rb0[LB::NR], rb1[LB::NR];
  int b_tp = 0, b_cc = 0;
  auto issue_b = [&](u32x4 (&rb)[LB::NR]) {
    lb.load(s_tap_kofs[b_tp] + b_cc * LMKD_BK, rb);
    if (++b_tp == ntap) { b_tp = 0; ++b_cc; }
  };
  int k_tp = 0, k_cc = 0;
  int k_sc = 0;
  bf16x8 av[NPL][NB / 2];
  auto step = [&](int t, u32x4 (&rb)[LB::NR], u32x4 (&rbn)[LB::NR]) {
    if (SRC2 ? k_tp == a.s2_t0[k_sc] : k_tp == 0) {
      __syncthreads();
      store_patch();
      __syncthreads();
      if constexpr (SRC2) {
        if (k_sc + 1 < a.s2_ncls) issue_patch(k_cc, k_sc + 1);
        else if (k_cc + 1 < a.cps) issue_patch(k_cc + 1, 0);
      } else {
        if (k_cc + 1 < a.cps) issue_patch(k_cc + 1);
      }
    }
    const uint2 pk2 = *reinterpret_cast<const uint2*>(adp_lane + k_tp * Cfg::BM);
    const unsigned ad[NB] = {((pk2.x & 0xffffu) << 4) + lane_off, ((pk2.x >> 16) << 4) + lane_off, ((pk2.y & 0xffffu) << 4) + lane_off,
                             ((pk2.y >> 16) << 4) + lane_off};
    constexpr int HB = NB / 2;
    auto read_a = [&](int hf) {
      if ((LMKD_ABL & 2) && t > 0) return;
#pragma unroll
      for (int p = 0; p < NPU; ++p)
#pragma unroll
        for (int b = 0; b < HB; ++b) av[p][b] = *reinterpret_cast<const bf16x8*>(psm + ad[hf * HB + b] + p * 64);
    };
    read_a(0);
    __builtin_amdgcn_sched_barrier(0);
#pragma unroll
    for (int hf = 0; hf < 2; ++hf) {
      if (hf == 1) {
        __builtin_amdgcn_sched_barrier(0);
        read_a(1);
        __builtin_amdgcn_sched_barrier(0);
      }
#pragma unroll
      for (int c = 0; c < NC; ++c) {
        const bf16x8 w0 = x3_as_bf16(rb[c * NPU + 0]), w1 = x3_as_bf16(rb[c * NPU + 1]), w2 = x3_as_bf16(rb[c * NPU + (NPU - 1)]);
#pragma unroll
        for (int b = 0; b < HB; ++b) {
          f32x4 d = acc[hf * HB + b][c];
          if constexpr (NPROD == 3) {
            d = __builtin_amdgcn_mfma_f32_16x16x32_f16(__builtin_bit_cast(f16x8, w1), __builtin_bit_cast(f16x8, av[0][b]), d, 0, 0, 0);
            d = __builtin_amdgcn_mfma_f32_16x16x32_f16(__builtin_bit_cast(f16x8, w0), __builtin_bit_cast(f16x8, av[1][b]), d, 0, 0, 0);
            d = __builtin_amdgcn_mfma_f32_16x16x32_f16(__builtin_bit_cast(f16x8, w0), __builtin_bit_cast(f16x8, av[0][b]), d, 0, 0, 0);
            acc[hf * HB + b][c] = d;
            continue;
          }
          if (NPROD == 9) {
            d = __builtin_amdgcn_mfma_f32_16x16x32_bf16(w2, av[2][b], d, 0, 0, 0);
            d = __builtin_amdgcn_mfma_f32_16x16x32_bf16(w2, av[1][b], d, 0, 0, 0);
            d = __builtin_amdgcn_mfma_f32_16x16x32_bf16(w1, av[2][b], d, 0, 0, 0);
          }
          d = __builtin_amdgcn_mfma_f32_16x16x32_bf16(w1, av[1][b], d, 0, 0, 0);
          d = __builtin_amdgcn_mfma_f32_16x16x32_bf16(w2, av[0][b], d, 0, 0, 0);
          d = __builtin_amdgcn_mfma_f32_16x16x32_bf16(w0, av[2][b], d, 0, 0, 0);
          d = __builtin_amdgcn_mfma_f32_16x16x32_bf16(w1, av[0][b], d, 0, 0, 0);
          d = __builtin_amdgcn_mfma_f32_16x16x32_bf16(w0, av[1][b], d, 0, 0, 0);
          d = __builtin_amdgcn_mfma_f32_16x16x32_bf16(w0, av[0][b], d, 0, 0, 0);
          acc[hf * HB + b][c] = d;
        }
      }
    }
    ++k_tp;
    if (SRC2 && k_sc + 1 < a.s2_ncls && k_tp == a.s2_t0[k_sc + 1]) ++k_sc;
    if (k_tp == ntap) { k_tp = 0; ++k_cc; k_sc = 0; k_cc_abl = 1; }
    __builtin_amdgcn_sched_barrier(0);
    x3_landed(rbn);
    x3_landed(rp);
    __builtin_amdgcn_sched_barrier(0);
    if (t + 2 < nk && !(LMKD_ABL & 1)) issue_b(rb);
  };
  if constexpr (EARLY) {
    if (nk > 0) issue_patch(0);
    patch16_fill_adp<Cfg, NB, ROWB>(s_adp, a, taps, ntap, tid, row0, M, halo, P);
  }
  __syncthreads();
  STAMP(1);
  if (nk > 0) {
    if (!EARLY) issue_patch(0);
    issue_b(rb0);
    if (nk > 1) issue_b(rb1);
    x3_landed(rp);
    x3_landed(rb0);
    x3_landed(rb1);
    __builtin_amdgcn_sched_barrier(0);
    STAMP(2);
    int t = 0;
    for (; t + 1 < nk; t += 2) {
      step(t, rb0, rb1);
      step(t + 1, rb1, rb0);
    }
    if (t < nk) step(t, rb0, rb1);
  }

  STAMP(3);
  const int ch0 = n0 + wn * (Cfg::TN * 32) + 4 * kq;
  float4 s1[NC], s2[NC];
  float amo = 0.f;
  float4 esc[NC], esh[NC];
  float4 bmean[NC], bistd[NC];
  constexpr bool bnb = BNB;
  const float* bnb_tab = bnb ? a.bnb_stats + (long)sg.seg * 5 * a.Co : nullptr;
#pragma unroll
  for (int c = 0; c < NC; ++c) {
    s1[c] = s2[c] = make_float4(0.f, 0.f, 0.f, 0.f);
    const int col = ch0 + 16 * c;
    const float4 z4 = make_float4(0.f, 0.f, 0.f, 0.f);
    if (EP || bnb) {
      const float* st = EP ? a.ep_stats : bnb_tab;
      esc[c] = col < a.Co ? *reinterpret_cast<const float4*>(st + 2 * a.Co + col) : z4;
      esh[c] = col < a.Co ? *reinterpret_cast<const float4*>(st + 3 * a.Co + col) : z4;
    }
    if (bnb) {
      bmean[c] = col < a.Co ? *reinterpret_cast<const float4*>(bnb_tab + col) : z4;
      bistd[c] = col < a.Co ? *reinterpret_cast<const float4*>(bnb_tab + a.Co + col) : z4;
    }
  }
#pragma unroll
  for (int b = 0; b < NB; ++b) {
    const int ob = s_out[wm * (Cfg::TM * 32) + 16 * b + pxl];
    float4 prev[NC];
    if (a.accum) {
#pragma unroll
      for (int c = 0; c < NC; ++c) {
        const int col = ch0 + 16 * c;
        prev[c] = (ob >= 0 && col < a.Co) ? *reinterpret_cast<const float4*>(a.out + (long)ob + col) : make_float4(0.f, 0.f, 0.f, 0.f);
      }
    }
#pragma unroll
// ... 72 lines not shown
```

lite-mkd_amd/csrc/conv_stem.h:

```cpp
#pragma once

#define STEM_MAX_WP 240

template <int NPROD, bool OUT16, int OR>
__global__ __launch_bounds__(256 * OR) void conv_stem_patch_kernel(ConvGemmArgs a) {
  constexpr int NPL = NPROD == 1 ? 1 : (NPROD == 3 ? 2 : 3);
  constexpr int NTHR = 256 * OR;
  using Cfg = X3Cfg<128 * OR, 64, 4 * OR, 1>;
  using LB = X3FragB<Cfg::TN, NPL>;
  constexpr int KH = 7, PR = 2 * (OR - 1) + KH;
  extern __shared__ __attribute__((aligned(16))) unsigned char psm[];
  __shared__ int s_out[Cfg::BM];
  __shared__ float s_red[Cfg::WM * Cfg::BN * 2];
  const int tid = threadIdx.x, lane = tid & 63, wave = tid >> 6;
  const int rt = blockIdx.x;
  const int pairs = (a.Ho + OR - 1) / OR;
  const int n = rt / pairs, oh0 = (rt - n * pairs) * OR;
  const int WP = a.halo;
  const int plane_bytes = PR * WP * 8;
  const int ih0 = 2 * oh0 - 3;
  float h2_sx = 1.f, h2_ix = 1.f, h2_iw = 1.f;
  const unsigned short* wpk = reinterpret_cast<const unsigned short*>(a.wpk);
  if constexpr (NPROD == 3) {
    const long nw = (long)a.Co * a.Kp;
    h2_sx = h2_scale(amax_read(a.h2_xw, (a.seg_m0 > 0 && (long)n * a.Ho * a.Wo >= a.seg_m0) ? 1 : 0));
    h2_ix = 1.f / h2_sx;
    h2_iw = 1.f / h2_scale(*reinterpret_cast<const unsigned*>(wpk + nw * 16));
    wpk += nw * 16 + 32;
  }
  {
    static_assert(STEM_MAX_WP <= 256, "one thread per patch column");
    constexpr int RSTEP = NTHR / 256, NIT = (PR + RSTEP - 1) / RSTEP;
    const __amdgpu_buffer_rsrc_t rs = x3_rsrc(a.src, (long)a.N * a.Hs * a.Ws * 16);
    const int pc = tid & 255, iw = pc - 3;
    u32x4 rp[NIT];
#pragma unroll
    for (int it = 0; it < NIT; ++it) {
      const int pr = (tid >> 8) + RSTEP * it, ih = ih0 + pr;
      const bool ok = pr < PR && (unsigned)ih < (unsigned)a.Hs && (unsigned)iw < (unsigned)a.Ws;
      rp[it] = __builtin_amdgcn_raw_buffer_load_b128(rs, ok ? (unsigned)(((n * a.Hs + ih) * a.Ws + iw) * 16) : X3_OOB, 0, 0);
    }
#pragma unroll
    for (int it = 0; it < NIT; ++it) {
      const int pr = (tid >> 8) + RSTEP * it;
      if (pr >= PR || pc >= WP) continue;
      const float4 v = make_float4(__uint_as_float(rp[it].x), __uint_as_float(rp[it].y), __uint_as_float(rp[it].z), __uint_as_float(rp[it].w));
      unsigned char* d = psm + (pr * WP + pc) * 8;
      if (NPL == 1) {
        *reinterpret_cast<uint2*>(d) = x3_round4(v);
      } else if constexpr (NPROD == 3) {
        uint2 q0, q1;
        h2_split4(v, h2_sx, q0, q1);
        *reinterpret_cast<uint2*>(d) = q0;
        *reinterpret_cast<uint2*>(d + plane_bytes) = q1;
      } else {
        uint2 q0, q1, q2;
        x3_split4(v, q0, q1, q2);
        *reinterpret_cast<uint2*>(d) = q0;
        *reinterpret_cast<uint2*>(d + plane_bytes) = q1;
        *reinterpret_cast<uint2*>(d + 2 * plane_bytes) = q2;
      }
    }
  }
  const int npix = OR * a.Wo;
  for (int r = tid; r < Cfg::BM; r += NTHR) {
    const int orow = r / a.Wo, ow = r - orow * a.Wo;
    s_out[r] = (r < npix && oh0 + orow < a.Ho) ? ((n * a.Ho + oh0 + orow) * a.Wo + ow) * a.Co : -1;
  }
  const int m = wave * 32 + (lane & 31);
  const bool active = __builtin_amdgcn_readfirstlane(wave * 32) < npix;
  int a_off = 0;
  {
    const int mm = m < npix ? m : 0;
    const int orow = mm / a.Wo, ow = mm - orow * a.Wo;
    a_off = ((2 * orow) * WP + 2 * ow + 2 * (lane >> 5)) * 8;
  }
  LB lb;
  lb.init(wpk, a.Co, a.Kp, 0, lane);
  f32x16 acc[1][Cfg::TN];
#pragma unroll
  for (int j = 0; j < Cfg::TN; ++j)
#pragma unroll
    for (int e = 0; e < 16; ++e) acc[0][j][e] = 0.f;
  u32x4 rb0[LB::NR], rb1[LB::NR];
  if (active) lb.load(0, rb0);
  __syncthreads();
  if (active) {
    auto step = [&](int kh, u32x4 (&rb)[LB::NR], u32x4 (&rbn)[LB::NR]) {
      if (kh + 1 < KH) lb.load((kh + 1) * 32, rbn);
      bf16x8 av[2][NPL];
#pragma unroll
      for (int g = 0; g < 2; ++g)
#pragma unroll
        for (int p = 0; p < NPL; ++p) av[g][p] = *reinterpret_cast<const bf16x8*>(psm + a_off + (kh * WP + 4 * g) * 8 + p * plane_bytes);
#pragma unroll
      for (int g = 0; g < 2; ++g)
#pragma unroll
        for (int j = 0; j < Cfg::TN; ++j) {
          f32x16 c = acc[0][j];
          if constexpr (NPROD == 1) {
            c = __builtin_amdgcn_mfma_f32_32x32x16_bf16(av[g][0], x3_as_bf16(rb[j * 2 + g]), c, 0, 0, 0);
          } else if constexpr (NPROD == 3) {
            const bf16x8 b0 = x3_as_bf16(rb[j * 4 + g * 2 + 0]), b1 = x3_as_bf16(rb[j * 4 + g * 2 + 1]);
            c = __builtin_amdgcn_mfma_f32_32x32x16_f16(__builtin_bit_cast(f16x8, av[g][1]), __builtin_bit_cast(f16x8, b0), c, 0, 0, 0);
            c = __builtin_amdgcn_mfma_f32_32x32x16_f16(__builtin_bit_cast(f16x8, av[g][0]), __builtin_bit_cast(f16x8, b1), c, 0, 0, 0);
            c = __builtin_amdgcn_mfma_f32_32x32x16_f16(__builtin_bit_cast(f16x8, av[g][0]), __builtin_bit_cast(f16x8, b0), c, 0, 0, 0);
          } else {
            const bf16x8 b0 = x3_as_bf16(rb[j * 6 + g * 3 + 0]), b1 = x3_as_bf16(rb[j * 6 + g * 3 + 1]), b2 = x3_as_bf16(rb[j * 6 + g * 3 + 2]);
            if (NPROD == 9) {
              c = __builtin_amdgcn_mfma_f32_32x32x16_bf16(av[g][2], b2, c, 0, 0, 0);
              c = __builtin_amdgcn_mfma_f32_32x32x16_bf16(av[g][1], b2, c, 0, 0, 0);
              c = __builtin_amdgcn_mfma_f32_32x32x16_bf16(av[g][2], b1, c, 0, 0, 0);
            }
            c = __builtin_amdgcn_mfma_f32_32x32x16_bf16(av[g][1], b1, c, 0, 0, 0);
            c = __builtin_amdgcn_mfma_f32_32x32x16_bf16(av[g][0], b2, c, 0, 0, 0);
            c = __builtin_amdgcn_mfma_f32_32x32x16_bf16(av[g][2], b0, c, 0, 0, 0);
            c = __builtin_amdgcn_mfma_f32_32x32x16_bf16(av[g][0], b1, c, 0, 0, 0);
            c = __builtin_amdgcn_mfma_f32_32x32x16_bf16(av[g][1], b0, c, 0, 0, 0);
            c = __builtin_amdgcn_mfma_f32_32x32x16_bf16(av[g][0], b0, c, 0, 0, 0);
          }
          acc[0][j] = c;
        }
    };
    step(0, rb0, rb1); step(1, rb1, rb0); step(2, rb0, rb1); step(3, rb1, rb0); step(4, rb0, rb1); step(5, rb1, rb0); step(6, rb0, rb1);
  }
#pragma unroll
  for (int e = 0; e < 16; ++e)
    if (s_out[wave * 32 + acc_row(e, lane)] < 0)
#pragma unroll
      for (int j = 0; j < Cfg::TN; ++j) acc[0][j][e] = 0.f;
  if constexpr (NPROD == 3) {
#pragma unroll
    for (int j = 0; j < Cfg::TN; ++j)
#pragma unroll
      for (int e = 0; e < 16; ++e) acc[0][j][e] = acc[0][j][e] * h2_ix * h2_iw;
  }
  x3_epilogue<Cfg, true, OUT16>(a, acc, s_out, s_red, rt, 0, wave, 0, lane, tid);
}
```

lite-mkd_amd/csrc/h2.h:

```cpp
#pragma once

typedef _Float16 f16x8 __attribute__((ext_vector_type(8)));
__device__ __forceinline__ float h2_scale(unsigned amax) {
  const int e = (int)((amax >> 23) & 0xffu) - 127 + ((amax & 0x7fffffu) ? 1 : 0);
  int s = 15 - e;
  s = s < -126 ? -126 : (s > 126 ? 126 : s);
  if (amax == 0u) s = 0;
  return __uint_as_float((unsigned)(s + 127) << 23);
}
typedef float f32x2_t __attribute__((ext_vector_type(2)));
typedef _Float16 f16x2_t __attribute__((ext_vector_type(2)));
__device__ __forceinline__ void h2_split4(const float4& v, float s, uint2& p0, uint2& p1) {
  union { f16x2_t h[2]; uint2 u; } c0, c1;
  const f32x2_t sv = {s, s};
  const f32x2_t xa = f32x2_t{v.x, v.y} * sv, xb = f32x2_t{v.z, v.w} * sv;
  c0.h[0] = __builtin_convertvector(xa, f16x2_t);
  c0.h[1] = __builtin_convertvector(xb, f16x2_t);
  c1.h[0] = __builtin_convertvector(xa - __builtin_convertvector(c0.h[0], f32x2_t), f16x2_t);
  c1.h[1] = __builtin_convertvector(xb - __builtin_convertvector(c0.h[1], f32x2_t), f16x2_t);
  p0 = c0.u;
  p1 = c1.u;
}
__device__ __forceinline__ void h2_split1(float x, unsigned short& p0, unsigned short& p1) {
  union { _Float16 h; unsigned short u; } c0, c1;
  c0.h = (_Float16)x;
  c1.h = (_Float16)(x - (float)c0.h);
  p0 = c0.u;
  p1 = c1.u;
}
```

lite-mkd_amd/csrc/wgrad_stem.h:

```cpp
#pragma once

struct StemWgradArgs {
  const float* dy;
  const float* x;
  float* slab;
  int N, H, W, Ho, Wo;
  int upi;
  int units, G, slabs;
  int RL;
  const unsigned* h2_xw;
  const unsigned* h2_dyw;
};

#define STEM_WG_LDA 160
#define STEM_WG_APLANE (32 * STEM_WG_LDA)

template <int V> struct StemSlot { static constexpr int value = V; };

template <int NPROD, int D, int RLC>
__global__ __launch_bounds__(512) void stem_wgrad_kernel(StemWgradArgs a) {
  static_assert(NPROD == 6 || NPROD == 9 || NPROD == 3, "three bf16 planes (6 / 9 products) or two fp16 planes (3 products: conv_patch16.h)");
  constexpr int NPL = NPROD == 3 ? 2 : 3;
  extern __shared__ __attribute__((aligned(16))) unsigned char smem[];
  const int RL = RLC ? RLC : a.RL;
  const int XBUF = 10 * NPL * RL;
  unsigned char* s_x = smem;
  unsigned char* s_dy = smem + 2 * XBUF;
  const int tid = threadIdx.x, lane = tid & 63, wave = tid >> 6;
  const int cb = wave & 3, nb = wave >> 2;
  const int q4 = lane >> 4, idx = lane & 15;
  const int W = a.W, Wo = a.Wo;

  for (int i = tid; i < (2 * XBUF) / 16; i += 512) reinterpret_cast<u32x4*>(s_x)[i] = u32x4{0u, 0u, 0u, 0u};

  const __amdgpu_buffer_rsrc_t rs_dy = x3_rsrc(a.dy, (long)a.N * a.Ho * Wo * 64 * 4);
  const __amdgpu_buffer_rsrc_t rs_x = x3_rsrc(a.x, (long)a.N * a.H * W * 4 * 4);

  float h2_sx = 1.f, h2_sdy = 1.f;
  if constexpr (NPROD == 3) {
    const unsigned mx0 = amax_read(a.h2_xw, 0), mx1 = amax_read(a.h2_xw, 1), md0 = amax_read(a.h2_dyw, 0), md1 = amax_read(a.h2_dyw, 1);
    h2_sx = h2_scale(mx0 > mx1 ? mx0 : mx1);
    h2_sdy = h2_scale(md0 > md1 ? md0 : md1);
  }
  const int d_k = tid >> 4, d_c = (tid & 15) * 4;
  u32x4 rq[D];
  u32x4 rx[9];
  auto as_f4 = [](const u32x4& r) { return make_float4(__uint_as_float(r.x), __uint_as_float(r.y), __uint_as_float(r.z), __uint_as_float(r.w)); };
  struct Pos { int u, ks, n, oh0, limit; };
  const int ksteps = (2 * Wo + 31) >> 5;
  auto set_unit = [&](Pos& p, int u) {
    p.u = u;
    p.ks = 0;
    if (u < 0) return;
    p.n = u / a.upi;
    p.oh0 = 2 * (u - p.n * a.upi);
    p.limit = (a.Ho - p.oh0 >= 2 ? 2 : 1) * Wo;
  };
  auto next_unit = [&](int u) {
    const int s = u / a.G;
    if (u + 1 < a.units && (u + 1) / a.G == s) return u + 1;
    const long ns = (long)s + gridDim.x;
    return ns < a.slabs ? (int)(ns * a.G) : -1;
  };
  auto load_dy = [&](u32x4& r, const Pos& p) {
    const int k = 32 * p.ks + d_k;
    r = __builtin_amdgcn_raw_buffer_load_b128(rs_dy, k < p.limit ? (unsigned)((((p.n * a.Ho + p.oh0) * Wo + k) * 64 + d_c) * 4) : X3_OOB, 0, 0);
  };
  auto load_x = [&](const Pos& p) {
#pragma unroll
    for (int j = 0; j < 9; ++j) {
      const int ih = 2 * p.oh0 - 3 + j;
      rx[j] = __builtin_amdgcn_raw_buffer_load_b128(rs_x, (tid < W && (unsigned)ih < (unsigned)a.H) ? (unsigned)((((p.n * a.H + ih) * W + tid) * 4) * 4) : X3_OOB, 0, 0);
    }
  };
  auto store_x = [&](int buf) {
    if (tid >= W) return;
    unsigned char* d = s_x + buf * XBUF + (tid + 3) * 8;
#pragma unroll
    for (int j = 0; j < 9; ++j) {
      uint2 p0, p1, p2;
      if constexpr (NPROD == 3) h2_split4(as_f4(rx[j]), h2_sx, p0, p1); else x3_split4(as_f4(rx[j]), p0, p1, p2);
      *reinterpret_cast<uint2*>(d + (j * NPL + 0) * RL) = p0;
      *reinterpret_cast<uint2*>(d + (j * NPL + 1) * RL) = p1;
      if constexpr (NPL == 3) *reinterpret_cast<uint2*>(d + (j * NPL + 2) * RL) = p2;
    }
  };

  const int a_off = (4 * q4 + (idx >> 2)) * STEM_WG_LDA + (16 * cb + 4 * (idx & 3)) * 2;
  const int b_col = 32 * nb + 8 * (idx & 3);
  f32x4 acc[7];
#pragma unroll
  for (int kh = 0; kh < 7; ++kh) acc[kh] = f32x4{0.f, 0.f, 0.f, 0.f};
  if ((int)blockIdx.x >= a.slabs) return;
  Pos cp, pf;
  set_unit(cp, (int)blockIdx.x * a.G);
  pf = cp;
  bool x_pending = false;
  auto advance_pf = [&]() {
    if (++pf.ks < ksteps) return;
    set_unit(pf, next_unit(pf.u));
    if (pf.u >= 0) {
      load_x(pf);
      x_pending = true;
    }
  };
  __syncthreads();
  load_x(cp);
  store_x(0);
#pragma unroll
  for (int d = 0; d < D; ++d) {
    if (pf.u >= 0) {
      load_dy(rq[d], pf);
      advance_pf();
    }
  }
  int xb = 0;
  int gstep = 0;
  auto step = [&](auto slot) {
    constexpr int S = decltype(slot)::value;
    if constexpr (NPROD == 3) tr_store4_h2<STEM_WG_LDA, STEM_WG_APLANE>(s_dy + (gstep & 1) * NPL * STEM_WG_APLANE, d_k, d_c, as_f4(rq[S]), h2_sdy);
    else tr_store4<NPL, STEM_WG_LDA, STEM_WG_APLANE>(s_dy + (gstep & 1) * NPL * STEM_WG_APLANE, d_k, d_c, as_f4(rq[S]));
    if (x_pending && cp.ks == ksteps - 1) {
      store_x(xb ^ 1);
      x_pending = false;
    }
    __syncthreads();
    if (pf.u >= 0) {
      load_dy(rq[S], pf);
      advance_pf();
    }
    const unsigned char* dyb = s_dy + (gstep & 1) * NPL * STEM_WG_APLANE;
    unsigned badr[2];
#pragma unroll
    for (int hh = 0; hh < 2; ++hh) {
      const int k = 32 * cp.ks + 16 * hh + 4 * q4 + (idx >> 2);
      const int r = k >= Wo ? 1 : 0;
      badr[hh] = (unsigned)(xb * XBUF + b_col + 2 * r * NPL * RL + 16 * (k - r * Wo));
    }
    bf16x8 fa[NPL];
#pragma unroll
    for (int p = 0; p < NPL; ++p) {
      const s16x4_t lo = __builtin_amdgcn_ds_read_tr16_b64_v4i16((s16x4_t __attribute__((address_space(3)))*)(dyb + p * STEM_WG_APLANE + a_off));
      const s16x4_t hi = __builtin_amdgcn_ds_read_tr16_b64_v4i16((s16x4_t __attribute__((address_space(3)))*)(dyb + p * STEM_WG_APLANE + a_off + 16 * STEM_WG_LDA));
      union { s16x4_t s[2]; bf16x8 b; } uu;
      uu.s[0] = lo; uu.s[1] = hi;
      fa[p] = uu.b;
    }
    bf16x8 fb[2][NPL];
    auto read_b = [&](int kh, bf16x8 (&f)[NPL]) {
#pragma unroll
      for (int p = 0; p < NPL; ++p) {
        const s16x4_t lo = __builtin_amdgcn_ds_read_tr16_b64_v4i16((s16x4_t __attribute__((address_space(3)))*)(s_x + badr[0] + (kh * NPL + p) * RL));
        const s16x4_t hi = __builtin_amdgcn_ds_read_tr16_b64_v4i16((s16x4_t __attribute__((address_space(3)))*)(s_x + badr[1] + (kh * NPL + p) * RL));
        union { s16x4_t s[2]; bf16x8 b; } uu;
        uu.s[0] = lo; uu.s[1] = hi;
        f[p] = uu.b;
      }
    };
    read_b(0, fb[0]);
#pragma unroll
    for (int kh = 0; kh < 7; ++kh) {
      if (kh + 1 < 7) read_b(kh + 1, fb[(kh + 1) & 1]);
      __builtin_amdgcn_sched_barrier(0);
      const bf16x8(&b)[NPL] = fb[kh & 1];
      f32x4 c = acc[kh];
      if constexpr (NPROD == 3) {
        c = __builtin_amdgcn_mfma_f32_16x16x32_f16(__builtin_bit_cast(f16x8, fa[1]), __builtin_bit_cast(f16x8, b[0]), c, 0, 0, 0);
        c = __builtin_amdgcn_mfma_f32_16x16x32_f16(__builtin_bit_cast(f16x8, fa[0]), __builtin_bit_cast(f16x8, b[1]), c, 0, 0, 0);
        c = __builtin_amdgcn_mfma_f32_16x16x32_f16(__builtin_bit_cast(f16x8, fa[0]), __builtin_bit_cast(f16x8, b[0]), c, 0, 0, 0);
      } else {
        if (NPROD == 9) {
          c = __builtin_amdgcn_mfma_f32_16x16x32_bf16(fa[NPL - 1], b[NPL - 1], c, 0, 0, 0);
          c = __builtin_amdgcn_mfma_f32_16x16x32_bf16(fa[1], b[NPL - 1], c, 0, 0, 0);
          c = __builtin_amdgcn_mfma_f32_16x16x32_bf16(fa[NPL - 1], b[1], c, 0, 0, 0);
        }
        c = __builtin_amdgcn_mfma_f32_16x16x32_bf16(fa[1], b[1], c, 0, 0, 0);
        c = __builtin_amdgcn_mfma_f32_16x16x32_bf16(fa[0], b[NPL - 1], c, 0, 0, 0);
        c = __builtin_amdgcn_mfma_f32_16x16x32_bf16(fa[NPL - 1], b[0], c, 0, 0, 0);
        c = __builtin_amdgcn_mfma_f32_16x16x32_bf16(fa[0], b[1], c, 0, 0, 0);
        c = __builtin_amdgcn_mfma_f32_16x16x32_bf16(fa[1], b[0], c, 0, 0, 0);
        c = __builtin_amdgcn_mfma_f32_16x16x32_bf16(fa[0], b[0], c, 0, 0, 0);
      }
      acc[kh] = c;
      __builtin_amdgcn_sched_barrier(0);
    }
    ++gstep;
    if (++cp.ks < ksteps) return;
    const int slab = cp.u / a.G;
    const int un = next_unit(cp.u);
    if (un < 0 || un / a.G != slab) {
      float* C = a.slab + (long)slab * 64 * 224;
#pragma unroll
      for (int kh = 0; kh < 7; ++kh) {
#pragma unroll
        for (int e = 0; e < 4; ++e)
          C[(16 * cb + 4 * q4 + e) * 224 + kh * 32 + 16 * nb + idx] = NPROD == 3 ? acc[kh][e] * (1.f / h2_sx) * (1.f / h2_sdy) : acc[kh][e];
        acc[kh] = f32x4{0.f, 0.f, 0.f, 0.f};
      }
    }
    set_unit(cp, un);
    xb ^= 1;
  };
  while (true) {
    step(StemSlot<0>());
    if (cp.u < 0) break;
    if constexpr (D > 1) {
      step(StemSlot<1>());
      if (cp.u < 0) break;
    }
    if constexpr (D > 2) {
      step(StemSlot<2>());
      if (cp.u < 0) break;
    }
    if constexpr (D > 3) {
      step(StemSlot<3>());
      if (cp.u < 0) break;
    }
    if constexpr (D > 4) {
      step(StemSlot<4>());
      if (cp.u < 0) break;
    }
    if constexpr (D > 5) {
      step(StemSlot<5>());
      if (cp.u < 0) break;
    }
  }
}
```

lite-mkd_amd/csrc/wgrad_win.h:

```cpp
#pragma once

struct WgradWinArgs {
  const float* dy;
  const float* x;
  float* slab;
  const float* pre_stats;
  int N, H, W, Cs, Co, Kp;
  int Mpix, steps_total, steps_per_split, splits;
  int n_ct, n_it;
  int seg_pix0, seg_splits0, sps1;
  FastDiv div_hw, div_w;
  const unsigned* h2_xw;
  const unsigned* h2_dyw;
};
template <int COB, int NPROD, bool ACT16, int R, bool PRE = false, int TPW = 9>
__global__ __launch_bounds__(64 * COB * ((9 + TPW - 1) / TPW)) void conv_wgrad_win_kernel(WgradWinArgs a) {
  constexpr int NPL = NPROD == 1 ? 1 : 3;
  static_assert(!ACT16 || (NPROD == 1 && !PRE), "bf16 tensors: one plane, no store-side arithmetic");
  constexpr int THREADS = 64 * COB * ((9 + TPW - 1) / TPW), BM = 32 * COB;
  constexpr int LDA = BM * 2 + 64, A_PLANE = LMKD_BK * LDA;
  constexpr int LDX = 64, X_PLANE = (R + 1) * LDX;
  constexpr int ESZ = ACT16 ? 2 : 4, EPL = ACT16 ? 8 : 4;
  constexpr int A_LPR = BM / EPL, A_RPP = THREADS / A_LPR, A_NI = (LMKD_BK + A_RPP - 1) / A_RPP;
  constexpr int X_LPR = 32 / EPL, X_RPP = THREADS / X_LPR, X_NI = (LMKD_BK + X_RPP - 1) / X_RPP;
// ... 20 lines not shown
  u32x4 ra[A_NI], rx[X_NI];
  unsigned x_ok = 0;
  float4 psc = float4(), psh = float4();
  if (PRE) {
    psc = *reinterpret_cast<const float4*>(a.pre_stats + (long)sl.seg * 5 * a.Cs + 2 * a.Cs + ci0 + x_c);
    psh = *reinterpret_cast<const float4*>(a.pre_stats + (long)sl.seg * 5 * a.Cs + 3 * a.Cs + ci0 + x_c);
  }
  auto load_dy = [&](int k0) {
#pragma unroll
    for (int i = 0; i < A_NI; ++i) {
      const int p = k0 + a_r + A_RPP * i;
      ra[i] = __builtin_amdgcn_raw_buffer_load_b128(rs_dy, (a_cin && a_r + A_RPP * i < LMKD_BK && p < kend) ? (unsigned)((p * a.Co + co0 + a_c) * ESZ) : X3_OOB, 0, 0);
    }
  };
  auto load_x = [&](int q0) {
#pragma unroll
    for (int i = 0; i < X_NI; ++i) {
      const int q = q0 + x_r + X_RPP * i;
      const bool ok = x_r + X_RPP * i < LMKD_BK && q >= 0 && q < a.Mpix;
      rx[i] = __builtin_amdgcn_raw_buffer_load_b128(rs_x, ok ? (unsigned)((q * a.Cs + ci0 + x_c) * ESZ) : X3_OOB, 0, 0);
      if (PRE) x_ok = ok ? (x_ok | (1u << i)) : (x_ok & ~(1u << i));
    }
  };
  auto as_f4 = [](const u32x4& r) { return make_float4(__uint_as_float(r.x), __uint_as_float(r.y), __uint_as_float(r.z), __uint_as_float(r.w)); };
  auto store_dy = [&]() {
#pragma unroll
    for (int i = 0; i < A_NI; ++i) {
      if (a_r + A_RPP * i >= LMKD_BK) continue;
      if constexpr (ACT16) tr_store8(s_dy, LDA, a_r + A_RPP * i, a_c, ra[i]);
      else tr_store4<NPL, LDA, A_PLANE>(s_dy, a_r + A_RPP * i, a_c, as_f4(ra[i]));
    }
  };
  auto store_x = [&](int q0) {
#pragma unroll
    for (int i = 0; i < X_NI; ++i) {
      if (x_r + X_RPP * i >= LMKD_BK) continue;
      const int slot = (q0 + x_r + X_RPP * i) & (R - 1);
      if constexpr (ACT16) {
        tr_store8(s_x, LDX, slot, x_c, rx[i]);
      } else {
        float4 v = as_f4(rx[i]);
        if (PRE && ((x_ok >> i) & 1u)) {
          v.x = fmaxf(fmaf(v.x, psc.x, psh.x), 0.f); v.y = fmaxf(fmaf(v.y, psc.y, psh.y), 0.f);
          v.z = fmaxf(fmaf(v.z, psc.z, psh.z), 0.f); v.w = fmaxf(fmaf(v.w, psc.w, psh.w), 0.f);
        }
        tr_store4<NPL, LDX, X_PLANE>(s_x, slot, x_c, v);
      }
    }
  };
  auto fill_adr = [&](unsigned* tab, int k0) {
    for (int e = tid; e < 9 * LMKD_BK; e += THREADS) {
      const int tp = e >> 5, r = e & 31;
      const int p = k0 + r;
      unsigned adr = (unsigned)(R * LDX);
      if (p < kend) {
        const int n = fdiv(p, a.div_hw);
        const int rem = p - n * a.H * a.W;
        const int h = fdiv(rem, a.div_w), w = rem - h * a.W;
        const int dh = tp / 3 - 1, dw = tp - (tp / 3) * 3 - 1;
        if ((unsigned)(h + dh) < (unsigned)a.H && (unsigned)(w + dw) < (unsigned)a.W) adr = (unsigned)(((p + dh * a.W + dw) & (R - 1)) * LDX);
      }
      tab[tp * LMKD_BK + ((((r >> 3) & 1) * 4 + (r & 3)) * 4 + ((r >> 4) * 2 + ((r >> 2) & 1)))] = adr;
    }
  };

  const int cb = (16 * ((lane >> 4) & 1) + 4 * (lane & 3)) * 2;
  const int cw = wave % COB, tap0 = (wave / COB) * TPW;
  const int offA = tr_lane_off(LDA, lane) + cw * 32 * 2;
  f32x16 acc[TPW];
#pragma unroll
  for (int t = 0; t < TPW; ++t)
#pragma unroll
    for (int e = 0; e < 16; ++e) acc[t][e] = 0.f;

  if (nk > 0) {
    const int kfirst = sl.kfirst;
    for (int j = tid; j < NPL * LDX / 4; j += THREADS)
      reinterpret_cast<unsigned*>(s_x + (j / (LDX / 4)) * X_PLANE + R * LDX)[j % (LDX / 4)] = 0u;
    for (int q0 = kfirst - halo; q0 < kfirst + halo; q0 += LMKD_BK) {
      load_x(q0);
      store_x(q0);
    }
    fill_adr(s_adr[0], kfirst);
    load_dy(kfirst);
    load_x(kfirst + halo);
    for (int t = 0; t < nk; ++t) {
      const int k0 = kfirst + t * LMKD_BK;
      store_dy();
      store_x(k0 + halo);
      __syncthreads();
      if (t + 1 < nk) {
        load_dy(k0 + LMKD_BK);
        load_x(k0 + LMKD_BK + halo);
        fill_adr(s_adr[(t + 1) & 1], k0 + LMKD_BK);
      }
      bf16x8 fa[2][NPL];
#pragma unroll
      for (int g = 0; g < 2; ++g)
#pragma unroll
        for (int p = 0; p < NPL; ++p) fa[g][p] = tr_frag<LDA>(s_dy, offA + p * A_PLANE + g * 16 * LDA);
#pragma unroll
      for (int ti = 0; ti < TPW; ++ti) {
        const int tp = tap0 + ti;
        if (9 % TPW != 0 && ti >= 9 - TPW * (9 / TPW) && tp >= 9) break;
        const u32x4 a4 = *reinterpret_cast<const u32x4*>(&s_adr[t & 1][tp * LMKD_BK + ((lane >> 5) * 4 + ((lane & 15) >> 2)) * 4]);
        f32x16 c = acc[ti];
#pragma unroll
        for (int g = 0; g < 2; ++g) {
          const unsigned ad[2] = {(g ? a4.z : a4.x) + (unsigned)cb, (g ? a4.w : a4.y) + (unsigned)cb};
          bf16x8 fb[NPL];
#pragma unroll
          for (int p = 0; p < NPL; ++p) {
            const s16x4_t lo = __builtin_amdgcn_ds_read_tr16_b64_v4i16((s16x4_t __attribute__((address_space(3)))*)(s_x + p * X_PLANE + ad[0]));
            const s16x4_t hi = __builtin_amdgcn_ds_read_tr16_b64_v4i16((s16x4_t __attribute__((address_space(3)))*)(s_x + p * X_PLANE + ad[1]));
            union { s16x4_t s[2]; bf16x8 b; } u;
            u.s[0] = lo; u.s[1] = hi;
            fb[p] = u.b;
          }
          if constexpr (NPROD == 1) {
            c = __builtin_amdgcn_mfma_f32_32x32x16_bf16(fa[g][0], fb[0], c, 0, 0, 0);
          } else {
            if (NPROD == 9) {
              c = __builtin_amdgcn_mfma_f32_32x32x16_bf16(fa[g][2], fb[2], c, 0, 0, 0);
              c = __builtin_amdgcn_mfma_f32_32x32x16_bf16(fa[g][1], fb[2], c, 0, 0, 0);
              c = __builtin_amdgcn_mfma_f32_32x32x16_bf16(fa[g][2], fb[1], c, 0, 0, 0);
            }
            c = __builtin_amdgcn_mfma_f32_32x32x16_bf16(fa[g][1], fb[1], c, 0, 0, 0);
            c = __builtin_amdgcn_mfma_f32_32x32x16_bf16(fa[g][0], fb[2], c, 0, 0, 0);
            c = __builtin_amdgcn_mfma_f32_32x32x16_bf16(fa[g][2], fb[0], c, 0, 0, 0);
            c = __builtin_amdgcn_mfma_f32_32x32x16_bf16(fa[g][0], fb[1], c, 0, 0, 0);
            c = __builtin_amdgcn_mfma_f32_32x32x16_bf16(fa[g][1], fb[0], c, 0, 0, 0);
            c = __builtin_amdgcn_mfma_f32_32x32x16_bf16(fa[g][0], fb[0], c, 0, 0, 0);
          }
        }
        acc[ti] = c;
      }
      __syncthreads();
    }
  }

  float* C = a.slab + (long)z * a.Co * a.Kp;
#pragma unroll
  for (int ti = 0; ti < TPW; ++ti) {
    if (9 % TPW != 0 && tap0 + ti >= 9) break;
    const int col = (tap0 + ti) * a.Cs + ci0 + (lane & 31);
#pragma unroll
    for (int e = 0; e < 16; ++e) {
      const int row = co0 + cw * 32 + acc_row(e, lane);
      if (row < a.Co) C[(long)row * a.Kp + col] = acc[ti][e];
    }
  }
}

template <int COB, int NPROD, int R, bool PRE = false, int TPW = 9, int JW = 2>
__global__ __launch_bounds__(64 * COB * ((9 + TPW - 1) / TPW) * (2 / JW), JW == 2 ? 2 : 3) void conv_wgrad_win16_kernel(WgradWinArgs a) {
  static_assert(JW == 2 || (JW == 1 && TPW == 9), "the channel-block split exists for nine taps per wave");
  static_assert(NPROD == 6 || NPROD == 9 || NPROD == 3, "three bf16 planes (6 / 9 products) or two fp16 planes (3 products: conv_patch16.h)");
  constexpr int NPL = NPROD == 3 ? 2 : 3;
  constexpr int THREADS = 64 * COB * ((9 + TPW - 1) / TPW) * (2 / JW), BM = 32 * COB;
  constexpr int LDA = BM * 2 + 32, A_PLANE = LMKD_BK * LDA;
  constexpr int LDX = 64, X_PLANE = (R + 1) * LDX;
  constexpr int A_LPR = BM / 4, A_RPP = THREADS / A_LPR, A_NI = (LMKD_BK + A_RPP - 1) / A_RPP;
  constexpr int X_LPR = 8, X_RPP = THREADS / X_LPR, X_NI = (LMKD_BK + X_RPP - 1) / X_RPP;
  static_assert(THREADS % A_LPR == 0 && THREADS % X_LPR == 0 && (LDA / 32) % 2 == 1, "tile layout");
  __shared__ __attribute__((aligned(16))) unsigned char s_dy[NPL * A_PLANE];
  __shared__ __attribute__((aligned(16))) unsigned char s_x[NPL * X_PLANE];
  __shared__ __attribute__((aligned(16))) unsigned s_adr[2][9 * LMKD_BK];
  const int tid = threadIdx.x, lane = tid & 63, wave = tid >> 6;
  const int tiles = a.n_ct * a.n_it;
  const int xj = blockIdx.x >> 3;
  const int z = (blockIdx.x & 7) + 8 * (xj / tiles);
  if (z >= a.splits) return;
  const int tz = xj - (xj / tiles) * tiles;
  const int co0 = (tz % a.n_ct) * BM, ci0 = (tz / a.n_ct) * 32;
  const WinSlab sl = win_slab(z, a.Mpix, a.steps_per_split, a.seg_pix0, a.seg_splits0, a.sps1);
  const int nk = sl.nk, kend = sl.kend;
  const int halo = a.W + 1;

  const __amdgpu_buffer_rsrc_t rs_dy = x3_rsrc(a.dy, (long)a.Mpix * a.Co * 4);
  const __amdgpu_buffer_rsrc_t rs_x = x3_rsrc(a.x, (long)a.Mpix * a.Cs * 4);
  const int a_c = (tid % A_LPR) * 4, a_r = tid / A_LPR;
  const bool a_cin = co0 + a_c < a.Co;
  const int x_c = (tid % X_LPR) * 4, x_r = tid / X_LPR;
  u32x4 ra[A_NI], rx[X_NI];
  unsigned x_ok = 0;
  float h2_sx = 1.f, h2_sdy = 1.f;
  if constexpr (NPROD == 3) {
    h2_sx = h2_scale(amax_read(a.h2_xw, sl.seg));
    h2_sdy = h2_scale(amax_read(a.h2_dyw, sl.seg));
  }
  float4 psc = float4(), psh = float4();
  if (PRE) {
    psc = *reinterpret_cast<const float4*>(a.pre_stats + (long)sl.seg * 5 * a.Cs + 2 * a.Cs + ci0 + x_c);
    psh = *reinterpret_cast<const float4*>(a.pre_stats + (long)sl.seg * 5 * a.Cs + 3 * a.Cs + ci0 + x_c);
  }
  auto load_dy = [&](int k0) {
#pragma unroll
    for (int i = 0; i < A_NI; ++i) {
      const int p = k0 + a_r + A_RPP * i;
      ra[i] = __builtin_amdgcn_raw_buffer_load_b128(rs_dy, (a_cin && a_r + A_RPP * i < LMKD_BK && p < kend) ? (unsigned)((p * a.Co + co0 + a_c) * 4) : X3_OOB, 0, 0);
    }
  };
  auto load_x = [&](int q0) {
#pragma unroll
    for (int i = 0; i < X_NI; ++i) {
      const int q = q0 + x_r + X_RPP * i;
      const bool ok = x_r + X_RPP * i < LMKD_BK && q >= 0 && q < a.Mpix;
      rx[i] = __builtin_amdgcn_raw_buffer_load_b128(rs_x, ok ? (unsigned)((q * a.Cs + ci0 + x_c) * 4) : X3_OOB, 0, 0);
      if (PRE) x_ok = ok ? (x_ok | (1u << i)) : (x_ok & ~(1u << i));
    }
  };
  auto as_f4 = [](const u32x4& r) { return make_float4(__uint_as_float(r.x), __uint_as_float(r.y), __uint_as_float(r.z), __uint_as_float(r.w)); };
  auto store_dy = [&]() {
#pragma unroll
    for (int i = 0; i < A_NI; ++i) {
      if (a_r + A_RPP * i >= LMKD_BK) continue;
      if constexpr (NPROD == 3) {
        uint2 p0, p1;
        h2_split4(as_f4(ra[i]), h2_sdy, p0, p1);
        unsigned char* d = s_dy + (a_r + A_RPP * i) * LDA + a_c * 2;
        *reinterpret_cast<uint2*>(d) = p0;
        *reinterpret_cast<uint2*>(d + A_PLANE) = p1;
      } else {
        tr_store4<NPL, LDA, A_PLANE>(s_dy, a_r + A_RPP * i, a_c, as_f4(ra[i]));
      }
    }
  };
  auto store_x = [&](int q0) {
#pragma unroll
    for (int i = 0; i < X_NI; ++i) {
      if (x_r + X_RPP * i >= LMKD_BK) continue;
      const int slot = (q0 + x_r + X_RPP * i) & (R - 1);
      float4 v = as_f4(rx[i]);
      if (PRE && ((x_ok >> i) & 1u)) {
        v.x = fmaxf(fmaf(v.x, psc.x, psh.x), 0.f); v.y = fmaxf(fmaf(v.y, psc.y, psh.y), 0.f);
        v.z = fmaxf(fmaf(v.z, psc.z, psh.z), 0.f); v.w = fmaxf(fmaf(v.w, psc.w, psh.w), 0.f);
      }
      uint2 p0, p1, p2;
      if constexpr (NPROD == 3) h2_split4(v, h2_sx, p0, p1); else x3_split4(v, p0, p1, p2);
      unsigned char* d = s_x + slot * LDX + ((x_c * 2) ^ (((slot >> 2) & 1) << 5));
      *reinterpret_cast<uint2*>(d) = p0;
      *reinterpret_cast<uint2*>(d + X_PLANE) = p1;
      if constexpr (NPL == 3) *reinterpret_cast<uint2*>(d + 2 * X_PLANE) = p2;
    }
  };
  auto fill_adr = [&](unsigned* tab, int k0) {
    for (int e = tid; e < 9 * LMKD_BK; e += THREADS) {
      const int tp = e >> 5, r = e & 31;
      const int p = k0 + r;
      unsigned adr = (unsigned)(R * LDX);
      if (p < kend) {
        const int n = fdiv(p, a.div_hw);
        const int rem = p - n * a.H * a.W;
        const int h = fdiv(rem, a.div_w), w = rem - h * a.W;
        const int dh = tp / 3 - 1, dw = tp - (tp / 3) * 3 - 1;
        if ((unsigned)(h + dh) < (unsigned)a.H && (unsigned)(w + dw) < (unsigned)a.W) {
          const int slot = (p + dh * a.W + dw) & (R - 1);
          adr = (unsigned)(slot * LDX + (((slot >> 2) & 1) << 5));
        }
      }
      tab[tp * LMKD_BK + (r & 15) * 2 + (r >> 4)] = adr;
    }
  };

  const int q4 = lane >> 4, idx = lane & 15;
  const int cw = wave % COB, tap0 = JW == 2 ? (wave / COB) * TPW : 0, j0 = JW == 2 ? 0 : wave / COB;
  const int offA = (4 * q4 + (idx >> 2)) * LDA + (cw * 32 + 4 * (idx & 3)) * 2;
  const unsigned cbx = (unsigned)(8 * (idx & 3));
  f32x4 acc[TPW][2][JW];
#pragma unroll
  for (int t = 0; t < TPW; ++t)
#pragma unroll
    for (int i = 0; i < 2; ++i)
#pragma unroll
      for (int j = 0; j < JW; ++j) acc[t][i][j] = f32x4{0.f, 0.f, 0.f, 0.f};

  if (nk > 0) {
    const int kfirst = sl.kfirst;
    for (int j = tid; j < NPL * LDX / 4; j += THREADS)
      reinterpret_cast<unsigned*>(s_x + (j / (LDX / 4)) * X_PLANE + R * LDX)[j % (LDX / 4)] = 0u;
    for (int q0 = kfirst - halo; q0 < kfirst + halo; q0 += LMKD_BK) {
      load_x(q0);
      store_x(q0);
    }
    fill_adr(s_adr[0], kfirst);
    load_dy(kfirst);
    load_x(kfirst + halo);
    for (int t = 0; t < nk; ++t) {
      const int k0 = kfirst + t * LMKD_BK;
      store_dy();
      store_x(k0 + halo);
      __syncthreads();
      if (t + 1 < nk) {
        load_dy(k0 + LMKD_BK);
        load_x(k0 + LMKD_BK + halo);
        fill_adr(s_adr[(t + 1) & 1], k0 + LMKD_BK);
      }
      bf16x8 fa[2][NPL];
#pragma unroll
      for (int i = 0; i < 2; ++i)
#pragma unroll
        for (int p = 0; p < NPL; ++p) {
          const unsigned char* ap = s_dy + p * A_PLANE + offA + i * 32;
          const s16x4_t lo = __builtin_amdgcn_ds_read_tr16_b64_v4i16((s16x4_t __attribute__((address_space(3)))*)ap);
          const s16x4_t hi = __builtin_amdgcn_ds_read_tr16_b64_v4i16((s16x4_t __attribute__((address_space(3)))*)(ap + 16 * LDA));
          union { s16x4_t s[2]; bf16x8 b; } u;
          u.s[0] = lo; u.s[1] = hi;
          fa[i][p] = u.b;
        }
      if constexpr (NPROD == 3 && JW == 2) {
        static_assert(NPROD != 3 || TPW == 9, "all nine taps per wave");
        auto read_fb = [&](int tp, bf16x8 (&fb)[JW][NPL]) {
          const uint2 a2 = *reinterpret_cast<const uint2*>(&s_adr[t & 1][tp * LMKD_BK + (4 * q4 + (idx >> 2)) * 2]);
#pragma unroll
          for (int j = 0; j < JW; ++j) {
            const unsigned lo_a = (a2.x ^ (unsigned)((j0 + j) << 5)) + cbx, hi_a = (a2.y ^ (unsigned)((j0 + j) << 5)) + cbx;
#pragma unroll
            for (int p = 0; p < NPL; ++p) {
              const s16x4_t lo = __builtin_amdgcn_ds_read_tr16_b64_v4i16((s16x4_t __attribute__((address_space(3)))*)(s_x + p * X_PLANE + lo_a));
              const s16x4_t hi = __builtin_amdgcn_ds_read_tr16_b64_v4i16((s16x4_t __attribute__((address_space(3)))*)(s_x + p * X_PLANE + hi_a));
              union { s16x4_t s[2]; bf16x8 b; } u;
              u.s[0] = lo; u.s[1] = hi;
              fb[j][p] = u.b;
            }
          }
        };
        auto mult = [&](int ti, const bf16x8 (&fb)[JW][NPL]) {
#pragma unroll
          for (int j = 0; j < JW; ++j)
#pragma unroll
            for (int i = 0; i < 2; ++i) {
              f32x4 c = acc[ti][i][j];
              c = __builtin_amdgcn_mfma_f32_16x16x32_f16(__builtin_bit_cast(f16x8, fa[i][1]), __builtin_bit_cast(f16x8, fb[j][0]), c, 0, 0, 0);
              c = __builtin_amdgcn_mfma_f32_16x16x32_f16(__builtin_bit_cast(f16x8, fa[i][0]), __builtin_bit_cast(f16x8, fb[j][1]), c, 0, 0, 0);
              c = __builtin_amdgcn_mfma_f32_16x16x32_f16(__builtin_bit_cast(f16x8, fa[i][0]), __builtin_bit_cast(f16x8, fb[j][0]), c, 0, 0, 0);
              acc[ti][i][j] = c;
            }
        };
        bf16x8 fb0[JW][NPL], fb1[JW][NPL];
        read_fb(tap0, fb0);
#pragma unroll
        for (int ti = 0; ti < TPW; ti += 2) {
          if (ti + 1 < TPW) read_fb(tap0 + ti + 1, fb1);
          mult(ti, fb0);
          if (ti + 1 < TPW) {
#pragma unroll
            for (int q = 0; q < JW * NPL * 2 + 1; ++q) {
              __builtin_amdgcn_sched_group_barrier(0x008, 1, 0);
              __builtin_amdgcn_sched_group_barrier(0x100, 1, 0);
            }
            __builtin_amdgcn_sched_group_barrier(0x008, JW * 6 - (JW * NPL * 2 + 1), 0);
            if (ti + 2 < TPW) read_fb(tap0 + ti + 2, fb0);
            mult(ti + 1, fb1);
            if (ti + 2 < TPW) {
#pragma unroll
              for (int q = 0; q < JW * NPL * 2 + 1; ++q) {
                __builtin_amdgcn_sched_group_barrier(0x008, 1, 0);
                __builtin_amdgcn_sched_group_barrier(0x100, 1, 0);
              }
              __builtin_amdgcn_sched_group_barrier(0x008, JW * 6 - (JW * NPL * 2 + 1), 0);
            }
          }
        }
      } else
#pragma unroll
      for (int ti = 0; ti < TPW; ++ti) {
        const int tp = tap0 + ti;
        if (9 % TPW != 0 && ti >= 9 - TPW * (9 / TPW) && tp >= 9) break;
        const uint2 a2 = *reinterpret_cast<const uint2*>(&s_adr[t & 1][tp * LMKD_BK + (4 * q4 + (idx >> 2)) * 2]);
#pragma unroll
        for (int j = 0; j < JW; ++j) {
          bf16x8 fb[NPL];
          const unsigned lo_a = (a2.x ^ (unsigned)((j0 + j) << 5)) + cbx, hi_a = (a2.y ^ (unsigned)((j0 + j) << 5)) + cbx;
#pragma unroll
          for (int p = 0; p < NPL; ++p) {
            const s16x4_t lo = __builtin_amdgcn_ds_read_tr16_b64_v4i16((s16x4_t __attribute__((address_space(3)))*)(s_x + p * X_PLANE + lo_a));
            const s16x4_t hi = __builtin_amdgcn_ds_read_tr16_b64_v4i16((s16x4_t __attribute__((address_space(3)))*)(s_x + p * X_PLANE + hi_a));
            union { s16x4_t s[2]; bf16x8 b; } u;
            u.s[0] = lo; u.s[1] = hi;
            fb[p] = u.b;
          }
#pragma unroll
          for (int i = 0; i < 2; ++i) {
            f32x4 c = acc[ti][i][j];
            if constexpr (NPROD == 3) {
              c = __builtin_amdgcn_mfma_f32_16x16x32_f16(__builtin_bit_cast(f16x8, fa[i][1]), __builtin_bit_cast(f16x8, fb[0]), c, 0, 0, 0);
              c = __builtin_amdgcn_mfma_f32_16x16x32_f16(__builtin_bit_cast(f16x8, fa[i][0]), __builtin_bit_cast(f16x8, fb[1]), c, 0, 0, 0);
              c = __builtin_amdgcn_mfma_f32_16x16x32_f16(__builtin_bit_cast(f16x8, fa[i][0]), __builtin_bit_cast(f16x8, fb[0]), c, 0, 0, 0);
              acc[ti][i][j] = c;
              continue;
            }
            if (NPROD == 9) {
              c = __builtin_amdgcn_mfma_f32_16x16x32_bf16(fa[i][NPL - 1], fb[NPL - 1], c, 0, 0, 0);
              c = __builtin_amdgcn_mfma_f32_16x16x32_bf16(fa[i][1], fb[NPL - 1], c, 0, 0, 0);
              c = __builtin_amdgcn_mfma_f32_16x16x32_bf16(fa[i][NPL - 1], fb[1], c, 0, 0, 0);
            }
            c = __builtin_amdgcn_mfma_f32_16x16x32_bf16(fa[i][1], fb[1], c, 0, 0, 0);
            c = __builtin_amdgcn_mfma_f32_16x16x32_bf16(fa[i][0], fb[NPL - 1], c, 0, 0, 0);
            c = __builtin_amdgcn_mfma_f32_16x16x32_bf16(fa[i][NPL - 1], fb[0], c, 0, 0, 0);
            c = __builtin_amdgcn_mfma_f32_16x16x32_bf16(fa[i][0], fb[1], c, 0, 0, 0);
            c = __builtin_amdgcn_mfma_f32_16x16x32_bf16(fa[i][1], fb[0], c, 0, 0, 0);
            c = __builtin_amdgcn_mfma_f32_16x16x32_bf16(fa[i][0], fb[0], c, 0, 0, 0);
            acc[ti][i][j] = c;
          }
        }
      }
      __syncthreads();
    }
  }

  float* C = a.slab + (long)z * a.Co * a.Kp;
  const float h2_ix = 1.f / h2_sx, h2_idy = 1.f / h2_sdy;
#pragma unroll
  for (int ti = 0; ti < TPW; ++ti) {
    if (9 % TPW != 0 && tap0 + ti >= 9) break;
#pragma unroll
    for (int i = 0; i < 2; ++i)
#pragma unroll
      for (int j = 0; j < JW; ++j) {
        const int col = (tap0 + ti) * a.Cs + ci0 + 16 * (j0 + j) + idx;
#pragma unroll
        for (int e = 0; e < 4; ++e) {
          const int row = co0 + cw * 32 + 16 * i + 4 * q4 + e;
          if (row < a.Co) C[(long)row * a.Kp + col] = NPROD == 3 ? acc[ti][i][j][e] * h2_ix * h2_idy : acc[ti][i][j][e];
        }
      }
  }
}
```

lite-mkd_amd/csrc/wgrad_x3.h:

```cpp
#pragma once

typedef short s16x4_t __attribute__((ext_vector_type(4)));

template <int BM_, int BN_, int WM_, int WN_>
struct WgCfg {
  static constexpr int BM = BM_, BN = BN_, WM = WM_, WN = WN_;
  static constexpr int TM = BM / WM / 32, TN = BN / WN / 32;
  static constexpr int THREADS = 64 * WM * WN;
  static_assert(TM >= 1 && TN >= 1 && WM * WN == 4, "4 waves");
};

template <int COLS>
struct TrImg {
  static constexpr int LDB = COLS * 2 + 64;
  static constexpr int PLANE = LMKD_BK * LDB;
  static_assert((LDB / 64) % 2 == 1, "row stride must be an odd multiple of 64 bytes");
};

template <int LDB>
__device__ __forceinline__ bf16x8 tr_frag(const unsigned char* __restrict__ img, int lane_off) {
  const unsigned char* a = img + lane_off;
  const s16x4_t lo = __builtin_amdgcn_ds_read_tr16_b64_v4i16((s16x4_t __attribute__((address_space(3)))*)a);
  const s16x4_t hi = __builtin_amdgcn_ds_read_tr16_b64_v4i16((s16x4_t __attribute__((address_space(3)))*)(a + 4 * LDB));
  union { s16x4_t s[2]; bf16x8 b; } u;
  u.s[0] = lo; u.s[1] = hi;
  return u.b;
}
__device__ __forceinline__ int tr_lane_off(int ldb, int lane) {
  const int idx = lane & 15;
  return (8 * (lane >> 5) + (idx >> 2)) * ldb + (16 * ((lane >> 4) & 1) + 4 * (idx & 3)) * 2;
}

template <int NPL, int LDB, int PLANE>
__device__ __forceinline__ void tr_store4(unsigned char* __restrict__ img, int k, int col, const float4& v) {
  unsigned char* d = img + k * LDB + col * 2;
  if (NPL == 1) {
    *reinterpret_cast<uint2*>(d) = x3_round4(v);
  } else {
    uint2 p0, p1, p2;
    x3_split4(v, p0, p1, p2);
    *reinterpret_cast<uint2*>(d) = p0;
    *reinterpret_cast<uint2*>(d + PLANE) = p1;
    *reinterpret_cast<uint2*>(d + 2 * PLANE) = p2;
  }
}

template <int LDB, int PLANE>
__device__ __forceinline__ void tr_store4_h2(unsigned char* __restrict__ img, int k, int col, const float4& v, float s) {
  unsigned char* d = img + k * LDB + col * 2;
  uint2 p0, p1;
  h2_split4(v, s, p0, p1);
  *reinterpret_cast<uint2*>(d) = p0;
  *reinterpret_cast<uint2*>(d + PLANE) = p1;
}

__device__ __forceinline__ void tr_store8(unsigned char* __restrict__ img, int ldb, int k, int col, const u32x4& v) {
  *reinterpret_cast<u32x4*>(img + k * ldb + col * 2) = v;
}

template <int ROWS, int THREADS>
struct LoaderMMajorDense16 {
  static constexpr int CPR = ROWS / 8, KPP = THREADS / CPR, NI = LMKD_BK / KPP;
  static_assert(THREADS % CPR == 0 && LMKD_BK % KPP == 0 && NI >= 1, "tile rows vs threads");
  const lmkd_bf16_t* base;
  long ld;
  u32x4 reg[NI];
  int K, r4;
  bool rin;
  __device__ __forceinline__ void init(const float* base_, long ld_, int row0, int nrows, int K_) {
    r4 = (threadIdx.x % CPR) * 8;
    rin = (row0 + r4) < nrows;
    base = reinterpret_cast<const lmkd_bf16_t*>(base_) + row0 + r4;
    ld = ld_; K = K_;
  }
  __device__ __forceinline__ void load(int koff) {
#pragma unroll
    for (int i = 0; i < NI; ++i) {
      const int k = koff + threadIdx.x / CPR + KPP * i;
      reg[i] = (rin && k < K) ? *reinterpret_cast<const u32x4*>(base + (long)k * ld) : u32x4{0u, 0u, 0u, 0u};
    }
  }
};
template <int ROWS, int THREADS>
struct LoaderWgradGather16 {
  static constexpr int CPR = ROWS / 8, KPP = THREADS / CPR, NI = LMKD_BK / KPP;
  const lmkd_bf16_t* x;
  FastDiv div_hw, div_w;
  int Mpix, HoWo, Wo, Hs, Ws, Cs, stride;
  u32x4 reg[NI];
  int dh, dw, coff, r4;
  bool tap_ok;
  unsigned inb;
  float4 psc, psh;
  __device__ __forceinline__ void init(const WgradArgs& a, int j0) {
    x = reinterpret_cast<const lmkd_bf16_t*>(a.x); div_hw = a.div_hw; div_w = a.div_w;
    Mpix = a.Mpix; HoWo = a.Ho * a.Wo; Wo = a.Wo; Hs = a.Hs; Ws = a.Ws; Cs = a.Cs; stride = a.stride;
    inb = 0u;
    r4 = (threadIdx.x % CPR) * 8;
    const int col = j0 + r4;
    const int tap = col / a.Cs;
    coff = col - tap * a.Cs;
    const int kh = tap / a.KWp, kw = tap - kh * a.KWp;
    dh = kh - a.pad; dw = kw - a.pad;
    tap_ok = col < a.Kp && kw < a.KW;
  }
  __device__ __forceinline__ void load(int koff) {
#pragma unroll
    for (int i = 0; i < NI; ++i) {
      const int p = koff + threadIdx.x / CPR + KPP * i;
      u32x4 v = {0u, 0u, 0u, 0u};
      if (tap_ok && p < Mpix) {
        const int n = fdiv(p, div_hw);
        const int rem = p - n * HoWo;
        const int oh = fdiv(rem, div_w);
        const int ow = rem - oh * Wo;
        const int h = oh * stride + dh, w = ow * stride + dw;
        if ((unsigned)h < (unsigned)Hs && (unsigned)w < (unsigned)Ws)
          v = *reinterpret_cast<const u32x4*>(x + ((long)(n * Hs + h) * Ws + w) * Cs + coff);
      }
      reg[i] = v;
    }
  }
};

template <class Cfg, bool SMALLC, int NPROD, bool PRE, bool ACT16 = false>
__global__ __launch_bounds__(Cfg::THREADS) void conv_wgrad_x3_kernel(WgradArgs a) {
  constexpr int NPL = NPROD == 1 ? 1 : (NPROD == 3 ? 2 : 3);
  static_assert(!ACT16 || (NPROD == 1 && !PRE), "bf16 activations: one plane, no store-side arithmetic");
  static_assert(NPROD != 3 || (!PRE && !SMALLC), "two-plane form: operands whose maxima their producers recorded");
  constexpr bool B16 = ACT16 && !SMALLC;
  using LA = typename std::conditional<ACT16, LoaderMMajorDense16<Cfg::BM, Cfg::THREADS>, LoaderMMajorDense<Cfg::BM, Cfg::THREADS>>::type;
  using LB = typename std::conditional<B16, LoaderWgradGather16<Cfg::BN, Cfg::THREADS>, LoaderWgradGather<Cfg::BN, SMALLC, Cfg::THREADS, PRE>>::type;
  using IA = TrImg<Cfg::BM>;
  using IB = TrImg<Cfg::BN>;
  constexpr int A_BYTES = NPL * IA::PLANE, B_BYTES = NPL * IB::PLANE;
  __shared__ __attribute__((aligned(16))) unsigned char smem[A_BYTES + B_BYTES];
  int z, tz;
  const int tiles_per_z = a.n_mt * a.n_jt;
  if (a.xcd_mode) {
    const int xj = blockIdx.x >> 3;
    z = (blockIdx.x & 7) + 8 * (xj / tiles_per_z);
    if (z >= a.splits) return;
    tz = xj - (xj / tiles_per_z) * tiles_per_z;
  } else {
    z = blockIdx.x / tiles_per_z;
    tz = blockIdx.x - z * tiles_per_z;
  }
  const int m0 = (tz % a.n_mt) * Cfg::BM, j0 = (tz / a.n_mt) * Cfg::BN;
  LA la;
  LB lb;
  const WinSlab sl = win_slab(z, a.Mpix, a.steps_per_split, a.seg_pix0, a.seg_splits0, a.sps1);
  const int nk = sl.nk, kb = sl.kfirst;
  la.init(a.dy, a.Co, m0, a.Co, sl.kend);
  lb.init(a, j0);
  lb.Mpix = sl.kend;
  if constexpr (PRE) {
    if (sl.seg && lb.tap_ok) {
      lb.psc = *reinterpret_cast<const float4*>(a.pre_stats + 5 * a.Cs + 2 * a.Cs + lb.coff);
      lb.psh = *reinterpret_cast<const float4*>(a.pre_stats + 5 * a.Cs + 3 * a.Cs + lb.coff);
    }
  }

  const int tid = threadIdx.x, lane = tid & 63, wave = tid >> 6;
  float h2_sx = 1.f, h2_sdy = 1.f;
  if constexpr (NPROD == 3) {
    h2_sx = h2_scale(amax_read(a.h2_xw, sl.seg));
    h2_sdy = h2_scale(amax_read(a.h2_dyw, sl.seg));
  }
  const int wm = wave / Cfg::WN, wn = wave % Cfg::WN;
  const int offA = tr_lane_off(IA::LDB, lane) + wm * (Cfg::TM * 32) * 2;
  const int offB = tr_lane_off(IB::LDB, lane) + wn * (Cfg::TN * 32) * 2;
  f32x16 acc[Cfg::TM][Cfg::TN];
#pragma unroll
  for (int i = 0; i < Cfg::TM; ++i)
#pragma unroll
    for (int j = 0; j < Cfg::TN; ++j)
#pragma unroll
      for (int e = 0; e < 16; ++e) acc[i][j][e] = 0.f;

  auto store_tiles = [&](unsigned char* sa, unsigned char* sb) {
#pragma unroll
    for (int i = 0; i < LA::NI; ++i) {
      if constexpr (ACT16) tr_store8(sa, IA::LDB, tid / LA::CPR + LA::KPP * i, la.r4, la.reg[i]);
      else if constexpr (NPROD == 3) tr_store4_h2<IA::LDB, IA::PLANE>(sa, tid / LA::CPR + LA::KPP * i, la.r4, la.reg[i], h2_sdy);
      else tr_store4<NPL, IA::LDB, IA::PLANE>(sa, tid / LA::CPR + LA::KPP * i, la.r4, la.reg[i]);
    }
    if constexpr (B16) {
#pragma unroll
      for (int i = 0; i < LB::NI; ++i) tr_store8(sb, IB::LDB, tid / LB::CPR + LB::KPP * i, lb.r4, lb.reg[i]);
    } else {
#pragma unroll
    for (int i = 0; i < LB::NI; ++i) {
      float4 v = lb.reg[i];
      if (PRE && ((lb.inb >> i) & 1u)) {
        v.x = fmaxf(fmaf(v.x, lb.psc.x, lb.psh.x), 0.f); v.y = fmaxf(fmaf(v.y, lb.psc.y, lb.psh.y), 0.f);
        v.z = fmaxf(fmaf(v.z, lb.psc.z, lb.psh.z), 0.f); v.w = fmaxf(fmaf(v.w, lb.psc.w, lb.psh.w), 0.f);
      }
      if constexpr (NPROD == 3) tr_store4_h2<IB::LDB, IB::PLANE>(sb, tid / LB::CPR + LB::KPP * i, lb.r4, v, h2_sx);
      else tr_store4<NPL, IB::LDB, IB::PLANE>(sb, tid / LB::CPR + LB::KPP * i, lb.r4, v);
    }
    }
  };
  auto kstep = [&](const unsigned char* sa, const unsigned char* sb) {
    bf16x8 fa[2][NPL][Cfg::TM], fb[2][NPL][Cfg::TN];
    auto read_group = [&](int g, bf16x8 (&xa)[NPL][Cfg::TM], bf16x8 (&xb)[NPL][Cfg::TN]) {
#pragma unroll
      for (int p = 0; p < NPL; ++p) {
#pragma unroll
        for (int i = 0; i < Cfg::TM; ++i) xa[p][i] = tr_frag<IA::LDB>(sa, offA + p * IA::PLANE + g * 16 * IA::LDB + i * 64);
#pragma unroll
        for (int j = 0; j < Cfg::TN; ++j) xb[p][j] = tr_frag<IB::LDB>(sb, offB + p * IB::PLANE + g * 16 * IB::LDB + j * 64);
      }
    };
    read_group(0, fa[0], fb[0]);
#pragma unroll
    for (int g = 0; g < 2; ++g) {
      if (g == 0) {
        read_group(1, fa[1], fb[1]);
        __builtin_amdgcn_sched_barrier(0);
      }
#pragma unroll
      for (int i = 0; i < Cfg::TM; ++i)
#pragma unroll
        for (int j = 0; j < Cfg::TN; ++j) {
          f32x16 c = acc[i][j];
          if constexpr (NPROD == 1) {
            c = __builtin_amdgcn_mfma_f32_32x32x16_bf16(fa[g][0][i], fb[g][0][j], c, 0, 0, 0);
          } else if constexpr (NPROD == 3) {
            c = __builtin_amdgcn_mfma_f32_32x32x16_f16(__builtin_bit_cast(f16x8, fa[g][1][i]), __builtin_bit_cast(f16x8, fb[g][0][j]), c, 0, 0, 0);
            c = __builtin_amdgcn_mfma_f32_32x32x16_f16(__builtin_bit_cast(f16x8, fa[g][0][i]), __builtin_bit_cast(f16x8, fb[g][1][j]), c, 0, 0, 0);
            c = __builtin_amdgcn_mfma_f32_32x32x16_f16(__builtin_bit_cast(f16x8, fa[g][0][i]), __builtin_bit_cast(f16x8, fb[g][0][j]), c, 0, 0, 0);
          } else {
            if (NPROD == 9) {
              c = __builtin_amdgcn_mfma_f32_32x32x16_bf16(fa[g][NPL - 1][i], fb[g][NPL - 1][j], c, 0, 0, 0);
              c = __builtin_amdgcn_mfma_f32_32x32x16_bf16(fa[g][1][i], fb[g][NPL - 1][j], c, 0, 0, 0);
              c = __builtin_amdgcn_mfma_f32_32x32x16_bf16(fa[g][NPL - 1][i], fb[g][1][j], c, 0, 0, 0);
            }
            c = __builtin_amdgcn_mfma_f32_32x32x16_bf16(fa[g][1][i], fb[g][1][j], c, 0, 0, 0);
            c = __builtin_amdgcn_mfma_f32_32x32x16_bf16(fa[g][0][i], fb[g][NPL - 1][j], c, 0, 0, 0);
            c = __builtin_amdgcn_mfma_f32_32x32x16_bf16(fa[g][NPL - 1][i], fb[g][0][j], c, 0, 0, 0);
            c = __builtin_amdgcn_mfma_f32_32x32x16_bf16(fa[g][0][i], fb[g][1][j], c, 0, 0, 0);
            c = __builtin_amdgcn_mfma_f32_32x32x16_bf16(fa[g][1][i], fb[g][0][j], c, 0, 0, 0);
            c = __builtin_amdgcn_mfma_f32_32x32x16_bf16(fa[g][0][i], fb[g][0][j], c, 0, 0, 0);
          }
          acc[i][j] = c;
        }
    }
  };

  if (nk > 0) {
    unsigned char* A0 = smem;
    unsigned char* B0 = smem + A_BYTES;
    la.load(kb);
    lb.load(kb);
    for (int t = 0; t < nk; ++t) {
      store_tiles(A0, B0);
      __syncthreads();
      if (t + 1 < nk) {
        la.load(kb + (t + 1) * LMKD_BK);
        lb.load(kb + (t + 1) * LMKD_BK);
      }
      kstep(A0, B0);
      __syncthreads();
    }
  }

  float* C = a.slab + (long)z * a.Co * a.Kp;
  const float h2_ix = 1.f / h2_sx, h2_idy = 1.f / h2_sdy;
#pragma unroll
  for (int j = 0; j < Cfg::TN; ++j) {
    const int col = j0 + wn * (Cfg::TN * 32) + j * 32 + (lane & 31);
    if (col >= a.Kp) continue;
#pragma unroll
    for (int i = 0; i < Cfg::TM; ++i)
#pragma unroll
      for (int e = 0; e < 16; ++e) {
        const int row = m0 + wm * (Cfg::TM * 32) + i * 32 + acc_row(e, lane);
        if (row < a.Co) C[(long)row * a.Kp + col] = NPROD == 3 ? acc[i][j][e] * h2_ix * h2_idy : acc[i][j][e];
      }
  }
}
```

Before: 51.74.

## Use mixed-precision FMA residual split, fold h2 scale into BN prologue, walk wgrad addresses

Replaces the fp16 hi/lo split (convert, convert back, subtract, convert) with a v_fma_mix instruction that computes the residual directly from the fp32 value, cutting ALU work in every tile staging path. In the window wgrad kernel, the per-tensor fp16 scale is folded into the BN scale/shift when a wave-wide check finds it exact, which removes a multiply per element. The address table fill replaces per-element fast divisions with an incremental h/w walk. Legacy toggles, per-config exceptions and probe entry points are added to compare the new paths against the old ones bit for bit. The new paths risk small rounding differences.

```diff
diff --git a/include/lmkd.h b/include/lmkd.h
--- a/include/lmkd.h
+++ b/include/lmkd.h
@@ -51,6 +51,11 @@
 int lmkd_conv_set_wgrad_win16(int on);
 int lmkd_conv_set_wgrad_stem(int on);
 int lmkd_conv_set_wgrad_window(int on);
+int lmkd_conv_set_wgrad_legacy(int on);
+int lmkd_h2_split_probe(const float* x, long n, float s, unsigned* sub_p0, unsigned* sub_p1, unsigned* mix_p0, unsigned* mix_p1, void* stream);
+int lmkd_h2_fold_probe(const float* x, const float* sc, const float* sh, long n, int C, float s, unsigned* ref_p0, unsigned* ref_p1,
+                       unsigned* fold_p0, unsigned* fold_p1, unsigned* folded, void* stream);
+int lmkd_wgrad_win_adr_probe(int N, int H, int W, int kfirst, int kend, int steps, int legacy, unsigned* out, void* stream);
 int lmkd_conv_set_patch16(int on);
 int lmkd_conv_set_persistent(int on);
 int lmkd_conv_set_xcd_mode(int mode);
diff --git a/lite-mkd_amd/csrc/capi.hip b/lite-mkd_amd/csrc/capi.hip
--- a/lite-mkd_amd/csrc/capi.hip
+++ b/lite-mkd_amd/csrc/capi.hip
@@ -1,4 +1,5 @@
 #include "common.h"
+#include "h2.h"
 #include <stdarg.h>
 
 static thread_local char g_err[512] = "";
@@ -35,3 +36,61 @@
   return LMKD_OK;
 }
 extern "C" int lmkd_get_activation_dtype(void) { return g_lmkd_act_bf16; }
+
+__global__ __launch_bounds__(256) void h2_split_probe_kernel(const float4* __restrict__ x, long n4, float s, uint2* sub0, uint2* sub1, uint2* mix0, uint2* mix1) {
+  for (long i = blockIdx.x * 256L + threadIdx.x; i < n4; i += gridDim.x * 256L) {
+    const float4 v = x[i];
+    uint2 a0, a1, b0, b1;
+    h2_split4_sub(v, s, a0, a1);
+    h2_split4(v, s, b0, b1);
+    sub0[i] = a0; sub1[i] = a1; mix0[i] = b0; mix1[i] = b1;
+  }
+}
+extern "C" int lmkd_h2_split_probe(const float* x, long n, float s, unsigned* sub_p0, unsigned* sub_p1, unsigned* mix_p0, unsigned* mix_p1, void* stream) {
+  LMKD_REQUIRE(x && sub_p0 && sub_p1 && mix_p0 && mix_p1 && n > 0 && n % 4 == 0, "lmkd_h2_split_probe: n must be a positive multiple of 4");
+  const long n4 = n / 4;
+  const int grid = (int)((n4 + 255) / 256 < 4096 ? (n4 + 255) / 256 : 4096);
+  hipLaunchKernelGGL(h2_split_probe_kernel, dim3(grid), dim3(256), 0, (hipStream_t)stream, (const float4*)x, n4, s, (uint2*)sub_p0, (uint2*)sub_p1,
+                     (uint2*)mix_p0, (uint2*)mix_p1);
+  LMKD_CHECK_LAUNCH("h2_split_probe_kernel");
+  return LMKD_OK;
+}
+__global__ __launch_bounds__(256) void h2_fold_probe_kernel(const float4* __restrict__ x, const float* __restrict__ sc, const float* __restrict__ sh, long n4, int C,
+                                                            float s, uint2* ref0, uint2* ref1, uint2* fold0, uint2* fold1, unsigned* folded) {
+  for (long i0 = blockIdx.x * 256L; i0 < n4; i0 += gridDim.x * 256L) {
+    const long i = i0 + threadIdx.x;
+    const bool in = i < n4;
+    const int c = (int)(((in ? i : 0) * 4) % C);
+    float4 psc = *reinterpret_cast<const float4*>(sc + c), psh = *reinterpret_cast<const float4*>(sh + c);
+    const float4 v = in ? x[i] : float4();
+    float4 y = make_float4(fmaxf(fmaf(v.x, psc.x, psh.x), 0.f), fmaxf(fmaf(v.y, psc.y, psh.y), 0.f), fmaxf(fmaf(v.z, psc.z, psh.z), 0.f),
+                           fmaxf(fmaf(v.w, psc.w, psh.w), 0.f));
+    uint2 a0, a1, b0, b1;
+    h2_split4_sub(y, s, a0, a1);
+    const bool fold = __all(h2_fold_ok(psc, psh, s));
+    if (fold) {
+      psc.x *= s; psc.y *= s; psc.z *= s; psc.w *= s;
+      psh.x *= s; psh.y *= s; psh.z *= s; psh.w *= s;
+      y = make_float4(fmaxf(fmaf(v.x, psc.x, psh.x), 0.f), fmaxf(fmaf(v.y, psc.y, psh.y), 0.f), fmaxf(fmaf(v.z, psc.z, psh.z), 0.f),
+                      fmaxf(fmaf(v.w, psc.w, psh.w), 0.f));
+      h2_split4_scaled(y, b0, b1);
+    } else {
+      h2_split4(y, s, b0, b1);
+    }
+    if (in) {
+      ref0[i] = a0; ref1[i] = a1; fold0[i] = b0; fold1[i] = b1;
+      if (fold) atomicAdd(folded, 1u);
+    }
+  }
+}
+extern "C" int lmkd_h2_fold_probe(const float* x, const float* sc, const float* sh, long n, int C, float s, unsigned* ref_p0, unsigned* ref_p1,
+                                  unsigned* fold_p0, unsigned* fold_p1, unsigned* folded, void* stream) {
+  LMKD_REQUIRE(x && sc && sh && ref_p0 && ref_p1 && fold_p0 && fold_p1 && folded && n > 0 && n % 4 == 0 && C > 0 && C % 4 == 0,
+               "lmkd_h2_fold_probe: n and C must be positive multiples of 4");
+  const long n4 = n / 4;
+  const int grid = (int)((n4 + 255) / 256 < 4096 ? (n4 + 255) / 256 : 4096);
+  hipLaunchKernelGGL(h2_fold_probe_kernel, dim3(grid), dim3(256), 0, (hipStream_t)stream, (const float4*)x, sc, sh, n4, C, s, (uint2*)ref_p0, (uint2*)ref_p1,
+                     (uint2*)fold_p0, (uint2*)fold_p1, folded);
+  LMKD_CHECK_LAUNCH("h2_fold_probe_kernel");
+  return LMKD_OK;
+}
diff --git a/lite-mkd_amd/csrc/conv.hip b/lite-mkd_amd/csrc/conv.hip
--- a/lite-mkd_amd/csrc/conv.hip
+++ b/lite-mkd_amd/csrc/conv.hip
@@ -1402,6 +1402,8 @@
 extern "C" int lmkd_conv_set_wgrad_planes(int on) { g_wgrad_planes = on ? 1 : 0; return LMKD_OK; }
 static int g_wgrad_win16 = 1;
 extern "C" int lmkd_conv_set_wgrad_win16(int on) { g_wgrad_win16 = on ? 1 : 0; return LMKD_OK; }
+static int g_wgrad_legacy = 0;
+extern "C" int lmkd_conv_set_wgrad_legacy(int on) { g_wgrad_legacy = on ? 1 : 0; return LMKD_OK; }
 static int g_wgrad_window = 1;
 extern "C" int lmkd_conv_set_wgrad_window(int on) { g_wgrad_window = on < 0 ? 0 : on; return LMKD_OK; }
 static inline bool wgrad_win_eligible(int W, int Cs, int Cout, int KH, int KW, int stride, int pad) {
@@ -1568,6 +1570,15 @@
     constexpr int JW = COB == 2 ? 1 : 2;
     constexpr int NT = 64 * COB * (2 / JW);
     with_nprod<3, 6, 9>(p.nprod, [&](auto np) {
+      if constexpr (decltype(np)::value == 3) {
+        if (g_wgrad_legacy) {
+          if (big && p.pre) hipLaunchKernelGGL((conv_wgrad_win16_kernel<COB, 3, 256, true, 9, JW, true>), grid, dim3(NT), 0, s, w);
+          else if (big) hipLaunchKernelGGL((conv_wgrad_win16_kernel<COB, 3, 256, false, 9, JW, true>), grid, dim3(NT), 0, s, w);
+          else if (p.pre) hipLaunchKernelGGL((conv_wgrad_win16_kernel<COB, 3, 128, true, 9, JW, true>), grid, dim3(NT), 0, s, w);
+          else hipLaunchKernelGGL((conv_wgrad_win16_kernel<COB, 3, 128, false, 9, JW, true>), grid, dim3(NT), 0, s, w);
+          return;
+        }
+      }
       if (big && p.pre) hipLaunchKernelGGL((conv_wgrad_win16_kernel<COB, np, 256, true, 9, JW>), grid, dim3(NT), 0, s, w);
       else if (big) hipLaunchKernelGGL((conv_wgrad_win16_kernel<COB, np, 256, false, 9, JW>), grid, dim3(NT), 0, s, w);
       else if (p.pre) hipLaunchKernelGGL((conv_wgrad_win16_kernel<COB, np, 128, true, 9, JW>), grid, dim3(NT), 0, s, w);
@@ -1765,3 +1776,33 @@
   info[4] = p.fam == ConvFam::Stem ? 2 : (p.fam == ConvFam::Patch || p.fam == ConvFam::Patch16 || p.fam == ConvFam::Patch1p ? 1 : 0);
   return LMKD_OK;
 }
+
+template <int R, bool LEGACY>
+__global__ __launch_bounds__(256) void win16_adr_probe_kernel(WgradWinArgs a, int kfirst, int kend, int steps, unsigned* out) {
+  __shared__ unsigned s_adr[9 * LMKD_BK];
+  Win16Adr<R, 256, LEGACY> adr;
+  adr.init(a);
+  adr.seek(a, kfirst);
+  for (int t = 0; t < steps; ++t) {
+    adr.fill(a, s_adr, kfirst + t * LMKD_BK, kend);
+    __syncthreads();
+    for (int e = threadIdx.x; e < 9 * LMKD_BK; e += 256) out[(long)t * 9 * LMKD_BK + e] = s_adr[e];
+    __syncthreads();
+  }
+}
+extern "C" int lmkd_wgrad_win_adr_probe(int N, int H, int W, int kfirst, int kend, int steps, int legacy, unsigned* out, void* stream) {
+  LMKD_REQUIRE(out && N > 0 && H > 0 && W > 0 && steps > 0 && kfirst >= 0 && kend <= N * H * W, "lmkd_wgrad_win_adr_probe: bad arguments");
+  LMKD_REQUIRE(32 + 2 * (W + 1) <= 256, "lmkd_wgrad_win_adr_probe: the window form exists for W <= 111");
+  WgradWinArgs w;
+  memset(&w, 0, sizeof(w));
+  w.N = N; w.H = H; w.W = W; w.Mpix = N * H * W;
+  w.div_hw = make_fastdiv(H * W); w.div_w = make_fastdiv(W);
+  const bool big = 32 + 2 * (W + 1) > 128;
+  hipStream_t s = (hipStream_t)stream;
+  if (big && legacy) hipLaunchKernelGGL((win16_adr_probe_kernel<256, true>), dim3(1), dim3(256), 0, s, w, kfirst, kend, steps, out);
+  else if (big) hipLaunchKernelGGL((win16_adr_probe_kernel<256, false>), dim3(1), dim3(256), 0, s, w, kfirst, kend, steps, out);
+  else if (legacy) hipLaunchKernelGGL((win16_adr_probe_kernel<128, true>), dim3(1), dim3(256), 0, s, w, kfirst, kend, steps, out);
+  else hipLaunchKernelGGL((win16_adr_probe_kernel<128, false>), dim3(1), dim3(256), 0, s, w, kfirst, kend, steps, out);
+  LMKD_CHECK_LAUNCH("win16_adr_probe_kernel");
+  return LMKD_OK;
+}
diff --git a/lite-mkd_amd/csrc/conv_patch.h b/lite-mkd_amd/csrc/conv_patch.h
--- a/lite-mkd_amd/csrc/conv_patch.h
+++ b/lite-mkd_amd/csrc/conv_patch.h
@@ -346,7 +346,7 @@
             *reinterpret_cast<uint2*>(d) = x3_round4(v);
           } else if constexpr (NPROD == 3) {
             uint2 q0, q1;
-            h2_split4(v, h2_sx, q0, q1);
+            if constexpr ((LMKD_H2_OLD & 1) || (PRE && Cfg::BM == 256 && Cfg::BN == 128)) h2_split4_sub(v, h2_sx, q0, q1); else h2_split4(v, h2_sx, q0, q1);
             *reinterpret_cast<uint2*>(d) = q0;
             *reinterpret_cast<uint2*>(d + 64) = q1;
           } else {
diff --git a/lite-mkd_amd/csrc/conv_patch16.h b/lite-mkd_amd/csrc/conv_patch16.h
--- a/lite-mkd_amd/csrc/conv_patch16.h
+++ b/lite-mkd_amd/csrc/conv_patch16.h
@@ -290,6 +290,7 @@
       uint2 q0, q1, q2;
       if constexpr (NPROD == 3) {
         if (LMKD_ABL & 4) { q0 = make_uint2(__float_as_uint(v.x), __float_as_uint(v.y)); q1 = make_uint2(__float_as_uint(v.z), __float_as_uint(v.w)); }
+        else if constexpr (LMKD_H2_OLD & 1) h2_split4_sub(v, h2_sx, q0, q1);
         else h2_split4(v, h2_sx, q0, q1);
       } else x3_split4(v, q0, q1, q2);
       *reinterpret_cast<uint2*>(d) = q0;
diff --git a/lite-mkd_amd/csrc/conv_stem.h b/lite-mkd_amd/csrc/conv_stem.h
--- a/lite-mkd_amd/csrc/conv_stem.h
+++ b/lite-mkd_amd/csrc/conv_stem.h
@@ -50,7 +50,7 @@
         *reinterpret_cast<uint2*>(d) = x3_round4(v);
       } else if constexpr (NPROD == 3) {
         uint2 q0, q1;
-        h2_split4(v, h2_sx, q0, q1);
+        if constexpr (LMKD_H2_OLD & 1) h2_split4_sub(v, h2_sx, q0, q1); else h2_split4(v, h2_sx, q0, q1);
         *reinterpret_cast<uint2*>(d) = q0;
         *reinterpret_cast<uint2*>(d + plane_bytes) = q1;
       } else {
diff --git a/lite-mkd_amd/csrc/h2.h b/lite-mkd_amd/csrc/h2.h
--- a/lite-mkd_amd/csrc/h2.h
+++ b/lite-mkd_amd/csrc/h2.h
@@ -1,5 +1,8 @@
 #pragma once
 
+#ifndef LMKD_H2_OLD
+#define LMKD_H2_OLD 0
+#endif
 typedef _Float16 f16x8 __attribute__((ext_vector_type(8)));
 __device__ __forceinline__ float h2_scale(unsigned amax) {
   const int e = (int)((amax >> 23) & 0xffu) - 127 + ((amax & 0x7fffffu) ? 1 : 0);
@@ -10,7 +13,7 @@
 }
 typedef float f32x2_t __attribute__((ext_vector_type(2)));
 typedef _Float16 f16x2_t __attribute__((ext_vector_type(2)));
-__device__ __forceinline__ void h2_split4(const float4& v, float s, uint2& p0, uint2& p1) {
+__device__ __forceinline__ void h2_split4_sub(const float4& v, float s, uint2& p0, uint2& p1) {
   union { f16x2_t h[2]; uint2 u; } c0, c1;
   const f32x2_t sv = {s, s};
   const f32x2_t xa = f32x2_t{v.x, v.y} * sv, xb = f32x2_t{v.z, v.w} * sv;
@@ -21,6 +24,43 @@
   p0 = c0.u;
   p1 = c1.u;
 }
+__device__ __forceinline__ unsigned h2_resid2(float x0, float x1, float s, unsigned h0) {
+  unsigned d;
+  asm("v_fma_mixlo_f16 %0, %1, %2, -%3 op_sel:[0,0,0] op_sel_hi:[0,0,1]" : "=v"(d) : "v"(x0), "v"(s), "v"(h0));
+  asm("v_fma_mixhi_f16 %0, %1, %2, -%3 op_sel:[0,0,1] op_sel_hi:[0,0,1]" : "+v"(d) : "v"(x1), "v"(s), "v"(h0));
+  return d;
+}
+__device__ __forceinline__ unsigned h2_resid2_scaled(float x0, float x1, unsigned h0) {
+  unsigned d;
+  asm("v_fma_mixlo_f16 %0, %1, 1.0, -%2 op_sel:[0,0,0] op_sel_hi:[0,0,1]" : "=v"(d) : "v"(x0), "v"(h0));
+  asm("v_fma_mixhi_f16 %0, %1, 1.0, -%2 op_sel:[0,0,1] op_sel_hi:[0,0,1]" : "+v"(d) : "v"(x1), "v"(h0));
+  return d;
+}
+__device__ __forceinline__ void h2_split4(const float4& v, float s, uint2& p0, uint2& p1) {
+  union { f16x2_t h[2]; uint2 u; } c0;
+  const f32x2_t sv = {s, s};
+  c0.h[0] = __builtin_convertvector(f32x2_t{v.x, v.y} * sv, f16x2_t);
+  c0.h[1] = __builtin_convertvector(f32x2_t{v.z, v.w} * sv, f16x2_t);
+  p0 = c0.u;
+  p1 = make_uint2(h2_resid2(v.x, v.y, s, c0.u.x), h2_resid2(v.z, v.w, s, c0.u.y));
+}
+__device__ __forceinline__ void h2_split4_scaled(const float4& v, uint2& p0, uint2& p1) {
+  union { f16x2_t h[2]; uint2 u; } c0;
+  c0.h[0] = __builtin_convertvector(f32x2_t{v.x, v.y}, f16x2_t);
+  c0.h[1] = __builtin_convertvector(f32x2_t{v.z, v.w}, f16x2_t);
+  p0 = c0.u;
+  p1 = make_uint2(h2_resid2_scaled(v.x, v.y, c0.u.x), h2_resid2_scaled(v.z, v.w, c0.u.y));
+}
+__device__ __forceinline__ bool h2_scaled_normal(float c, float s) {
+  const int e = (int)((__float_as_uint(c) >> 23) & 0xffu), es = (int)((__float_as_uint(s) >> 23) & 0xffu) - 127;
+  return (c == 0.f) || (e >= 1 && e <= 254 && e + es >= 1 && e + es <= 254);
+}
+__device__ __forceinline__ bool h2_fold_ok(const float4& sc, const float4& sh, float s) {
+  const int es = (int)((__float_as_uint(s) >> 23) & 0xffu) - 127;
+  return es <= 64 && es >= -126 &&
+         h2_scaled_normal(sc.x, s) && h2_scaled_normal(sc.y, s) && h2_scaled_normal(sc.z, s) && h2_scaled_normal(sc.w, s) &&
+         h2_scaled_normal(sh.x, s) && h2_scaled_normal(sh.y, s) && h2_scaled_normal(sh.z, s) && h2_scaled_normal(sh.w, s);
+}
 __device__ __forceinline__ void h2_split1(float x, unsigned short& p0, unsigned short& p1) {
   union { _Float16 h; unsigned short u; } c0, c1;
   c0.h = (_Float16)x;
diff --git a/lite-mkd_amd/csrc/wgrad_stem.h b/lite-mkd_amd/csrc/wgrad_stem.h
--- a/lite-mkd_amd/csrc/wgrad_stem.h
+++ b/lite-mkd_amd/csrc/wgrad_stem.h
@@ -79,7 +79,8 @@
 #pragma unroll
     for (int j = 0; j < 9; ++j) {
       uint2 p0, p1, p2;
-      if constexpr (NPROD == 3) h2_split4(as_f4(rx[j]), h2_sx, p0, p1); else x3_split4(as_f4(rx[j]), p0, p1, p2);
+      if constexpr (NPROD == 3 && (LMKD_H2_OLD & 2)) h2_split4_sub(as_f4(rx[j]), h2_sx, p0, p1);
+      else if constexpr (NPROD == 3) h2_split4(as_f4(rx[j]), h2_sx, p0, p1); else x3_split4(as_f4(rx[j]), p0, p1, p2);
       *reinterpret_cast<uint2*>(d + (j * NPL + 0) * RL) = p0;
       *reinterpret_cast<uint2*>(d + (j * NPL + 1) * RL) = p1;
       if constexpr (NPL == 3) *reinterpret_cast<uint2*>(d + (j * NPL + 2) * RL) = p2;
diff --git a/lite-mkd_amd/csrc/wgrad_win.h b/lite-mkd_amd/csrc/wgrad_win.h
--- a/lite-mkd_amd/csrc/wgrad_win.h
+++ b/lite-mkd_amd/csrc/wgrad_win.h
@@ -196,7 +196,60 @@
   }
 }
 
-template <int COB, int NPROD, int R, bool PRE = false, int TPW = 9, int JW = 2>
+template <int R, int THREADS, bool LEGACY>
+struct Win16Adr {
+  static constexpr int LDX = 64;
+  bool walk;
+  unsigned rcp;
+  int h0, w0;
+  __device__ __forceinline__ void init(const WgradWinArgs& a) {
+    walk = !LEGACY && a.W >= 7 && a.H >= 5;
+    rcp = fdiv(65535u, a.div_w) + 1u;
+    h0 = w0 = 0;
+  }
+  __device__ __forceinline__ void seek(const WgradWinArgs& a, int k0) {
+    if (!walk) return;
+    const int n = fdiv(k0, a.div_hw);
+    const int rem = k0 - n * a.H * a.W;
+    h0 = fdiv(rem, a.div_w);
+    w0 = rem - h0 * a.W;
+  }
+  __device__ __forceinline__ void fill(const WgradWinArgs& a, unsigned* tab, int k0, int kend) {
+    for (int e = threadIdx.x; e < 9 * LMKD_BK; e += THREADS) {
+      const int tp = e >> 5, r = e & 31;
+      const int p = k0 + r;
+      unsigned adr = (unsigned)(R * LDX);
+      if (p < kend) {
+        int h, w;
+        if (walk) {
+          const unsigned wr = (unsigned)(w0 + r), q = __umul24(wr, rcp) >> 16;
+          const unsigned hq = (unsigned)h0 + q;
+          w = (int)(wr - __umul24(q, (unsigned)a.W));
+          h = (int)min(hq, hq - (unsigned)a.H);
+        } else {
+          const int n = fdiv(p, a.div_hw);
+          const int rem = p - n * a.H * a.W;
+          h = fdiv(rem, a.div_w);
+          w = rem - h * a.W;
+        }
+        const int dh = tp / 3 - 1, dw = tp - (tp / 3) * 3 - 1;
+        if ((unsigned)(h + dh) < (unsigned)a.H && (unsigned)(w + dw) < (unsigned)a.W) {
+          const int slot = (p + dh * a.W + dw) & (R - 1);
+          adr = (unsigned)(slot * LDX + (((slot >> 2) & 1) << 5));
+        }
+      }
+      tab[tp * LMKD_BK + (r & 15) * 2 + (r >> 4)] = adr;
+    }
+    if (walk) {
+      const unsigned wr = (unsigned)(w0 + LMKD_BK), q = (wr * rcp) >> 16;
+      const unsigned hq = (unsigned)h0 + q;
+      w0 = (int)(wr - q * (unsigned)a.W);
+      h0 = (int)min(hq, hq - (unsigned)a.H);
+    }
+  }
+};
+
+template <int COB, int NPROD, int R, bool PRE = false, int TPW = 9, int JW = 2, bool LEGACY = false>
 __global__ __launch_bounds__(64 * COB * ((9 + TPW - 1) / TPW) * (2 / JW), JW == 2 ? 2 : 3) void conv_wgrad_win16_kernel(WgradWinArgs a) {
   static_assert(JW == 2 || (JW == 1 && TPW == 9), "the channel-block split exists for nine taps per wave");
   static_assert(NPROD == 6 || NPROD == 9 || NPROD == 3, "three bf16 planes (6 / 9 products) or two fp16 planes (3 products: conv_patch16.h)");
@@ -238,6 +291,14 @@
     psc = *reinterpret_cast<const float4*>(a.pre_stats + (long)sl.seg * 5 * a.Cs + 2 * a.Cs + ci0 + x_c);
     psh = *reinterpret_cast<const float4*>(a.pre_stats + (long)sl.seg * 5 * a.Cs + 3 * a.Cs + ci0 + x_c);
   }
+  bool fold = false;
+  if constexpr (PRE && NPROD == 3 && !LEGACY && !(LMKD_H2_OLD & 12)) {
+    fold = __all(h2_fold_ok(psc, psh, h2_sx));
+    if (fold) {
+      psc.x *= h2_sx; psc.y *= h2_sx; psc.z *= h2_sx; psc.w *= h2_sx;
+      psh.x *= h2_sx; psh.y *= h2_sx; psh.z *= h2_sx; psh.w *= h2_sx;
+    }
+  }
   auto load_dy = [&](int k0) {
 #pragma unroll
     for (int i = 0; i < A_NI; ++i) {
@@ -261,7 +322,7 @@
       if (a_r + A_RPP * i >= LMKD_BK) continue;
       if constexpr (NPROD == 3) {
         uint2 p0, p1;
-        h2_split4(as_f4(ra[i]), h2_sdy, p0, p1);
+        if constexpr (LEGACY || (LMKD_H2_OLD & 4)) h2_split4_sub(as_f4(ra[i]), h2_sdy, p0, p1); else h2_split4(as_f4(ra[i]), h2_sdy, p0, p1);
         unsigned char* d = s_dy + (a_r + A_RPP * i) * LDA + a_c * 2;
         *reinterpret_cast<uint2*>(d) = p0;
         *reinterpret_cast<uint2*>(d + A_PLANE) = p1;
@@ -281,31 +342,18 @@
         v.z = fmaxf(fmaf(v.z, psc.z, psh.z), 0.f); v.w = fmaxf(fmaf(v.w, psc.w, psh.w), 0.f);
       }
       uint2 p0, p1, p2;
-      if constexpr (NPROD == 3) h2_split4(v, h2_sx, p0, p1); else x3_split4(v, p0, p1, p2);
+      if constexpr (NPROD == 3 && (LEGACY || (LMKD_H2_OLD & 4))) h2_split4_sub(v, h2_sx, p0, p1);
+      else if constexpr (NPROD == 3) { if (PRE && fold) h2_split4_scaled(v, p0, p1); else h2_split4(v, h2_sx, p0, p1); }
+      else x3_split4(v, p0, p1, p2);
       unsigned char* d = s_x + slot * LDX + ((x_c * 2) ^ (((slot >> 2) & 1) << 5));
       *reinterpret_cast<uint2*>(d) = p0;
       *reinterpret_cast<uint2*>(d + X_PLANE) = p1;
       if constexpr (NPL == 3) *reinterpret_cast<uint2*>(d + 2 * X_PLANE) = p2;
     }
   };
-  auto fill_adr = [&](unsigned* tab, int k0) {
-    for (int e = tid; e < 9 * LMKD_BK; e += THREADS) {
-      const int tp = e >> 5, r = e & 31;
-      const int p = k0 + r;
-      unsigned adr = (unsigned)(R * LDX);
-      if (p < kend) {
-        const int n = fdiv(p, a.div_hw);
-        const int rem = p - n * a.H * a.W;
-        const int h = fdiv(rem, a.div_w), w = rem - h * a.W;
-        const int dh = tp / 3 - 1, dw = tp - (tp / 3) * 3 - 1;
-        if ((unsigned)(h + dh) < (unsigned)a.H && (unsigned)(w + dw) < (unsigned)a.W) {
-          const int slot = (p + dh * a.W + dw) & (R - 1);
-          adr = (unsigned)(slot * LDX + (((slot >> 2) & 1) << 5));
-        }
-      }
-      tab[tp * LMKD_BK + (r & 15) * 2 + (r >> 4)] = adr;
-    }
-  };
+  Win16Adr<R, THREADS, LEGACY || NPROD != 3 || (LMKD_H2_OLD & 16)> adr;
+  adr.init(a);
+  auto fill_adr = [&](unsigned* tab, int k0) { adr.fill(a, tab, k0, kend); };
 
   const int q4 = lane >> 4, idx = lane & 15;
   const int cw = wave % COB, tap0 = JW == 2 ? (wave / COB) * TPW : 0, j0 = JW == 2 ? 0 : wave / COB;
@@ -327,6 +375,7 @@
       load_x(q0);
       store_x(q0);
     }
+    adr.seek(a, kfirst);
     fill_adr(s_adr[0], kfirst);
     load_dy(kfirst);
     load_x(kfirst + halo);
diff --git a/lite-mkd_amd/csrc/wgrad_x3.h b/lite-mkd_amd/csrc/wgrad_x3.h
--- a/lite-mkd_amd/csrc/wgrad_x3.h
+++ b/lite-mkd_amd/csrc/wgrad_x3.h
@@ -45,11 +45,11 @@
   }
 }
 
-template <int LDB, int PLANE>
+template <int LDB, int PLANE, bool MIX = true>
 __device__ __forceinline__ void tr_store4_h2(unsigned char* __restrict__ img, int k, int col, const float4& v, float s) {
   unsigned char* d = img + k * LDB + col * 2;
   uint2 p0, p1;
-  h2_split4(v, s, p0, p1);
+  if constexpr (MIX && !(LMKD_H2_OLD & 2)) h2_split4(v, s, p0, p1); else h2_split4_sub(v, s, p0, p1);
   *reinterpret_cast<uint2*>(d) = p0;
   *reinterpret_cast<uint2*>(d + PLANE) = p1;
 }
@@ -178,11 +178,12 @@
 #pragma unroll
       for (int e = 0; e < 16; ++e) acc[i][j][e] = 0.f;
 
+  constexpr bool H2MIX = !(Cfg::BM == 128 && Cfg::BN == 64);
   auto store_tiles = [&](unsigned char* sa, unsigned char* sb) {
 #pragma unroll
     for (int i = 0; i < LA::NI; ++i) {
       if constexpr (ACT16) tr_store8(sa, IA::LDB, tid / LA::CPR + LA::KPP * i, la.r4, la.reg[i]);
-      else if constexpr (NPROD == 3) tr_store4_h2<IA::LDB, IA::PLANE>(sa, tid / LA::CPR + LA::KPP * i, la.r4, la.reg[i], h2_sdy);
+      else if constexpr (NPROD == 3) tr_store4_h2<IA::LDB, IA::PLANE, H2MIX>(sa, tid / LA::CPR + LA::KPP * i, la.r4, la.reg[i], h2_sdy);
       else tr_store4<NPL, IA::LDB, IA::PLANE>(sa, tid / LA::CPR + LA::KPP * i, la.r4, la.reg[i]);
     }
     if constexpr (B16) {
@@ -196,7 +197,7 @@
         v.x = fmaxf(fmaf(v.x, lb.psc.x, lb.psh.x), 0.f); v.y = fmaxf(fmaf(v.y, lb.psc.y, lb.psh.y), 0.f);
         v.z = fmaxf(fmaf(v.z, lb.psc.z, lb.psh.z), 0.f); v.w = fmaxf(fmaf(v.w, lb.psc.w, lb.psh.w), 0.f);
       }
-      if constexpr (NPROD == 3) tr_store4_h2<IB::LDB, IB::PLANE>(sb, tid / LB::CPR + LB::KPP * i, lb.r4, v, h2_sx);
+      if constexpr (NPROD == 3) tr_store4_h2<IB::LDB, IB::PLANE, H2MIX>(sb, tid / LB::CPR + LB::KPP * i, lb.r4, v, h2_sx);
       else tr_store4<NPL, IB::LDB, IB::PLANE>(sb, tid / LB::CPR + LB::KPP * i, lb.r4, v);
     }
     }
```

Measured after the change: 51.14. 0.989x the previous value.
